# DomhnallBoyle/lip2speech-unit

Measured on AMD Instinct MI355X. Metric: real-time factor (audio-sec/wall-sec), end-to-end lip->16kHz audio, 4s@25fps clips, higher is better.
Workload: dtype fp16; 1 GPU; e2e lip->units->wav (BASELINE configs[3]: AV-HuBERT large 24L + conformer 12x512 + multi_input HiFi-GAN), 4-s 100-frame 88x88 clips, batch 640 per GPU; clips_per_gpu=640, streams=1, clips_per_launch=640, frames_per_clip=100, hipgraph=True, input=uint8 96x96 frames resident in HBM, crop+normalise on device, enc_layers=24, conf_layers=12, parallelism=clip-parallel dp1

## Files before the change

include/lip2speech_hip.h:

```cpp
#ifndef LIP2SPEECH_HIP_H
#define LIP2SPEECH_HIP_H

#include <stddef.h>
#include <stdint.h>

#ifdef __cplusplus
extern "C" {
#endif

#define L2S_ABI_VERSION 16

enum { L2S_F16 = 0, L2S_BF16 = 1, L2S_F32 = 2 };

enum { L2S_OK = 0, L2S_EINVAL = -1, L2S_ESHAPE = -2, L2S_EALIGN = -3, L2S_EUNSUPPORTED = -4 };

enum {
  L2S_ACT_NONE = 0,
  L2S_ACT_RELU = 1,
  L2S_ACT_GELU = 2,
  L2S_ACT_SWISH = 3,
  L2S_ACT_PRELU = 4,
  L2S_ACT_LRELU = 5,
  L2S_ACT_TANH = 6
};

enum {
  L2S_F_RES_PRE  = 1 << 0,
  L2S_F_RES_POST = 1 << 1,
  L2S_F_ACCUM    = 1 << 2,
  L2S_F_DUAL     = 1 << 3,
  L2S_F_MASK     = 1 << 4,
  L2S_F_OUT_F32  = 1 << 5,
  L2S_F_RES_F32  = 1 << 6
};

enum {
  L2S_MODE_LINEAR = 0,
  L2S_MODE_CONV1D = 1,
  L2S_MODE_CONV2D = 2
};

typedef struct l2s_gemm_desc {
  const void* A;
  const void* W;
  void* C;
  void* C2;
  const float* bias;
  const float* slope;
  const void* R;
  const int32_t* lens;
  int32_t M, N, Cin, ntaps;
  int32_t lda, ldc, ldc2, ldr;
  int32_t mode;
  int32_t T_out, T_in, stride, dil, off;
  int32_t Ho, Wo, Hi, Wi, KW, pad;
  int32_t out_row_mul, out_row_add;
  int32_t mask_T, mask_mul;
  int32_t act, flags, dtype;
  float alpha;
  float act_slope;
  float slope2;
  int32_t groups, a_gstride, c_gstride;
  int64_t w_gstride;
  const int32_t* ktab;
} l2s_gemm_desc;
#define L2S_KTAB_MAX 9

int l2s_abi_version(void);
const char* l2s_build_info(void);

int l2s_tapgemm(const l2s_gemm_desc* host_desc, void* stream);
#define L2S_VARIANT_F32 2128128
int l2s_tapgemm_variant(const l2s_gemm_desc* host_desc);
#define L2S_EPI_FAMILY_F32 32
int l2s_tapgemm_epilogue_family(const l2s_gemm_desc* host_desc);

int l2s_stem_conv3d(const void* x, int x_is_f32, const void* w, const float* bias, const float* slope,
                    void* y, int B, int T, int H, int W, int dtype, void* stream);

int l2s_stem_pool_fused(const void* x, int x_is_f32, const void* w, const float* bias, const float* slope,
                        void* y, int B, int T, int H, int W, int dtype, void* stream);

int l2s_stem_pool_fused_u8(const uint8_t* frames, int Hin, int Win, int crop, float mean, float std, const void* w,
                           const float* bias, const float* slope, void* y, int B, int T, int dtype, void* stream);

int l2s_maxpool2d_3x3s2(const void* x, void* y, int N, int H, int W, int C, int dtype, void* stream);

int l2s_avgpool_hw(const void* x, void* y, int N, int HW, int C, int dtype, void* stream);

int l2s_layernorm(const void* x, int x_is_f32, int ldx, const float* gamma, const float* beta, float eps,
                  void* y, int y_is_f32, int ldy, void* y2, int ldy2, int M, int C, int zero_prefix,
                  const int32_t* lens, int len_mul, int mask_T, int dtype, void* stream);

int l2s_attention(const void* qkv, int ldq, void* out, int ldo, const void* pos, int ldp,
                  const float* bias_u, const float* bias_v, const int32_t* lens, int len_mul,
                  int B, int T, int H, int dtype, void* stream);

int l2s_glu_dwconv_swish(const void* x, const float* w, const float* bias, void* y, const int32_t* lens,
                         int len_mul, int B, int T, int C, int k, int dtype, void* stream);

int l2s_greedy_decode(const float* logits, int ldl, const int32_t* lens, int len_mul, int B, int T2, int V,
                      float temperature, float lenpen, int32_t* tokens, float* lprobs, float* score, void* stream);

int l2s_beam_decode(const float* logits, int ldl, const int32_t* lens, int len_mul, int B, int T2, int V, float temperature,
                    float lenpen, int beam, void* workspace, size_t workspace_bytes, int32_t* tokens, float* pos_scores,
                    float* score, int32_t* nhyp, void* stream);
size_t l2s_beam_decode_workspace(int B, int T2, int beam);

int l2s_ctc_frames(const float* logits, int ldl, const int32_t* lens, int len_mul, int B, int L, int V, int K, int32_t* labels,
                   int32_t* topk_cls, float* topk_lp, void* stream);

int l2s_ctc_beam_search(const int32_t* topk_cls, const float* topk_lp, const int32_t* lens, int len_mul, int B, int L, int K,
                        int beam, int nbest, void* workspace, size_t workspace_bytes, int32_t* labels, int32_t* lengths,
                        float* scores, void* stream);
size_t l2s_ctc_beam_workspace(int B, int L, int beam);
int l2s_ctc_repeat_labels(const int32_t* x, int ldx, const int32_t* lens, int len_mul, int B, int L, int32_t* y, int ldy,
                          void* stream);

int l2s_repeat2_cast(const float* x, void* y, int B, int T, int C, int dtype, void* stream);

int l2s_splitk_reduce(const float* P, int ldp, int S, float* x, int ldx, int M, int N, void* stream);

int l2s_splitk_reduce_layernorm(const float* P, int ldp, int S, float* x, int ldx, const float* gamma, const float* beta, float eps,
                                void* y, int y_is_f32, int ldy, int M, int C, const int32_t* lens, int len_mul, int mask_T,
                                int dtype, void* stream);

int l2s_cast_f32_to_16(const float* x, int ldx, void* y, int ldy, int M, int C, int dtype, void* stream);
int l2s_cast_16_to_f32(const void* x, int ldx, float* y, int ldy, int M, int C, int dtype, void* stream);
int l2s_broadcast_rows(const void* v, int ldv, void* y, int ldy, int col0, const int32_t* lens, int len_mul,
                       int B, int T, int C, int v_is_f32, int dtype, void* stream);
int l2s_transpose_ct_to_tc(const float* x, void* y, int ldy, int col0, const int32_t* lens, int len_mul,
                           int B, int C, int T, int dtype, void* stream);
int l2s_embedding(const int32_t* code, const void* table, void* y, int ldy, const int32_t* lens,
                  int B, int L, int C, int dtype, void* stream);
int l2s_embedding_tokens(const int32_t* tok, int ldt, int token_offset, const void* table, int n_rows, void* y, int ldy,
                         const int32_t* lens, int len_mul, int B, int L, int C, int dtype, void* stream);
int l2s_rows_f32_to_16_masked(const float* x, int ldx, void* y, int ldy, int col0, const int32_t* lens, int len_mul,
                              int B, int T, int C, int dtype, void* stream);
int l2s_lens_from_mask(const uint8_t* mask, int32_t* lens, int B, int T, void* stream);
int l2s_split_hi_lo(const float* x, int ldx, void* hi, void* lo, int ld16, int act, float slope, const int32_t* lens,
                    int len_mul, int B, int T, int C, int dtype, void* stream);

typedef struct l2s_respair_desc {
  const void* X; const void* W1; const void* W2; const float* b1; const float* b2;
  void* Y; float* XS; const int32_t* lens;
  int32_t len_mul, B, T, C, k, dil, last, accumulate, dtype;
  float slope;
} l2s_respair_desc;
int l2s_respair(const l2s_respair_desc* d, void* stream);

typedef struct l2s_respair_final_desc {
  const void* X[3]; const void* W1[3]; const void* W2[3]; const float* b1[3]; const float* b2[3];
  int32_t k[3], dil[3];
  void* Y; const int32_t* lens;
  int32_t n, len_mul, B, T, C, dtype;
  float slope;
} l2s_respair_final_desc;
int l2s_respair_final(const l2s_respair_final_desc* d, void* stream);

int l2s_basicblock_fused(const void* x, const void* w1, const float* b1, const float* s1, const void* w2, const float* b2,
                         const float* s2, void* y, int n_images, int H, int W, int C, int dtype, void* stream);
int l2s_basiclayer_fused(const void* x, const void* const* w, const float* const* bias, const float* const* slope, int n_blocks,
                         void* y, int n_images, int H, int W, int C, int dtype, void* stream);
int l2s_basicstage128_tail_fused(const void* x0, const void* t0, const void* wa, const float* ba, const float* sa, const void* w1,
                                 const float* b1, const float* s1, const void* w2, const float* b2, const float* s2, void* y,
                                 int n_images, int H, int W, int dtype, void* stream);

int l2s_conv_post_tanh(const float* x, const float* w, float bias, float* wav, int16_t* pcm, const int32_t* lens,
                       int len_mul, int B, int T, int C, int k, void* stream);

int l2s_resblock_fused(const void* xl, const void* w, const float* bias, float* xs, void* xl_out,
                       const int32_t* lens, int len_mul, int B, int T, int C, int k, int d0, int d1, int d2,
                       int accumulate, float slope, int dtype, void* stream);

int l2s_resstage_fused(const void* xl, const void* const* w, const float* const* bias, const int* ks, const int* dils,
                       int n_blocks, float* xs, void* xl_out, const int32_t* lens, int len_mul, int B, int T, int C,
                       float slope, int xs_final, int dtype, void* stream);

int l2s_preprocess_frames(const uint8_t* frames, void* y, int B, int T, int Hin, int Win, int crop, float mean,
                          float std, int dtype, void* stream);

int l2s_mel_spectrogram(const void* wav, int wav_is_i16, int64_t ldw, const int32_t* n_samples, int B, int S, const float* basis,
                        const float* fb, const int32_t* fb_range, float* mel, int ldm, int T_rows, int n_fft, int hop,
                        int n_mels, float floor_, void* stream);

int l2s_unit_ce(const float* logits, int ldl, const int32_t* target, int ldt, const int32_t* lens, int len_mul, int B, int T2,
                int V, int pad_idx, int ignore_prefix, float* nll, float* smooth, int32_t* n_correct, int32_t* n_tok,
                void* stream);
int l2s_mel_l1_sc(const float* pred, int Tm_pred, const float* targ, int Tm_targ, const int32_t* lens, int len_mul, int B,
                  int n_mels, int crop_len, float* l1, float* sq, float* tsq, int32_t* n_rows, void* stream);
size_t l2s_ctc_loss_workspace(int B, int L, int S_max);
int l2s_ctc_loss(const float* logits, int ldl, const int32_t* lens, int len_mul, int B, int L, int V, int blank,
                 const int32_t* targets, const int32_t* tgt_lens, const int32_t* tgt_offs, int S_max, void* workspace,
                 size_t workspace_bytes, float* nll, void* stream);

#ifdef __cplusplus
}
#endif
#endif
```

lip2speech_unit_amd/_lib.py:

```python
import ctypes
import os

_HERE = os.path.dirname(os.path.abspath(__file__))
LIB_PATH = os.environ.get("L2S_LIB_PATH") or os.path.join(_HERE, "liblip2speech_hip.so")

F16, BF16, F32 = 0, 1, 2
ACT_NONE, ACT_RELU, ACT_GELU, ACT_SWISH, ACT_PRELU, ACT_LRELU, ACT_TANH = range(7)
F_RES_PRE, F_RES_POST, F_ACCUM, F_DUAL, F_MASK, F_OUT_F32, F_RES_F32 = (1 << i for i in range(7))
MODE_LINEAR, MODE_CONV1D, MODE_CONV2D = 0, 1, 2
ABI_VERSION = 16

_ERR = {-1: "L2S_EINVAL", -2: "L2S_ESHAPE", -3: "L2S_EALIGN", -4: "L2S_EUNSUPPORTED"}


class L2SError(RuntimeError):
    pass


class GemmDesc(ctypes.Structure):
    _fields_ = [
        ("A", ctypes.c_void_p), ("W", ctypes.c_void_p), ("C", ctypes.c_void_p), ("C2", ctypes.c_void_p),
        ("bias", ctypes.c_void_p), ("slope", ctypes.c_void_p), ("R", ctypes.c_void_p), ("lens", ctypes.c_void_p),
        ("M", ctypes.c_int32), ("N", ctypes.c_int32), ("Cin", ctypes.c_int32), ("ntaps", ctypes.c_int32),
        ("lda", ctypes.c_int32), ("ldc", ctypes.c_int32), ("ldc2", ctypes.c_int32), ("ldr", ctypes.c_int32),
        ("mode", ctypes.c_int32),
        ("T_out", ctypes.c_int32), ("T_in", ctypes.c_int32), ("stride", ctypes.c_int32), ("dil", ctypes.c_int32),
        ("off", ctypes.c_int32),
        ("Ho", ctypes.c_int32), ("Wo", ctypes.c_int32), ("Hi", ctypes.c_int32), ("Wi", ctypes.c_int32),
        ("KW", ctypes.c_int32), ("pad", ctypes.c_int32),
        ("out_row_mul", ctypes.c_int32), ("out_row_add", ctypes.c_int32),
        ("mask_T", ctypes.c_int32), ("mask_mul", ctypes.c_int32),
        ("act", ctypes.c_int32), ("flags", ctypes.c_int32), ("dtype", ctypes.c_int32),
        ("alpha", ctypes.c_float), ("act_slope", ctypes.c_float), ("slope2", ctypes.c_float),
        ("groups", ctypes.c_int32), ("a_gstride", ctypes.c_int32), ("c_gstride", ctypes.c_int32),
        ("w_gstride", ctypes.c_int64),
        ("ktab", ctypes.c_void_p),
    ]


_vp, _i, _f = ctypes.c_void_p, ctypes.c_int, ctypes.c_float


class RespairDesc(ctypes.Structure):
    _fields_ = [("X", ctypes.c_void_p), ("W1", ctypes.c_void_p), ("W2", ctypes.c_void_p), ("b1", ctypes.c_void_p),
                ("b2", ctypes.c_void_p), ("Y", ctypes.c_void_p), ("XS", ctypes.c_void_p), ("lens", ctypes.c_void_p),
                ("len_mul", ctypes.c_int32), ("B", ctypes.c_int32), ("T", ctypes.c_int32), ("C", ctypes.c_int32),
                ("k", ctypes.c_int32), ("dil", ctypes.c_int32), ("last", ctypes.c_int32), ("accumulate", ctypes.c_int32),
                ("dtype", ctypes.c_int32), ("slope", ctypes.c_float)]


class RespairFinalDesc(ctypes.Structure):
    _fields_ = [("X", ctypes.c_void_p * 3), ("W1", ctypes.c_void_p * 3), ("W2", ctypes.c_void_p * 3), ("b1", ctypes.c_void_p * 3),
                ("b2", ctypes.c_void_p * 3), ("k", ctypes.c_int32 * 3), ("dil", ctypes.c_int32 * 3),
                ("Y", ctypes.c_void_p), ("lens", ctypes.c_void_p),
                ("n", ctypes.c_int32), ("len_mul", ctypes.c_int32), ("B", ctypes.c_int32), ("T", ctypes.c_int32),
                ("C", ctypes.c_int32), ("dtype", ctypes.c_int32), ("slope", ctypes.c_float)]


SIGNATURES = {
    "l2s_abi_version": ([], ctypes.c_int),
    "l2s_build_info": ([], ctypes.c_char_p),
    "l2s_tapgemm": ([ctypes.POINTER(GemmDesc), _vp], _i),
    "l2s_tapgemm_variant": ([ctypes.POINTER(GemmDesc)], _i),
    "l2s_tapgemm_epilogue_family": ([ctypes.POINTER(GemmDesc)], _i),
    "l2s_stem_conv3d": ([_vp, _i, _vp, _vp, _vp, _vp, _i, _i, _i, _i, _i, _vp], _i),
    "l2s_stem_pool_fused": ([_vp, _i, _vp, _vp, _vp, _vp, _i, _i, _i, _i, _i, _vp], _i),
    "l2s_stem_pool_fused_u8": ([_vp, _i, _i, _i, _f, _f, _vp, _vp, _vp, _vp, _i, _i, _i, _vp], _i),
    "l2s_maxpool2d_3x3s2": ([_vp, _vp, _i, _i, _i, _i, _i, _vp], _i),
    "l2s_avgpool_hw": ([_vp, _vp, _i, _i, _i, _i, _vp], _i),
    "l2s_layernorm": ([_vp, _i, _i, _vp, _vp, _f, _vp, _i, _i, _vp, _i, _i, _i, _i, _vp, _i, _i, _i, _vp], _i),
    "l2s_attention": ([_vp, _i, _vp, _i, _vp, _i, _vp, _vp, _vp, _i, _i, _i, _i, _i, _vp], _i),
    "l2s_glu_dwconv_swish": ([_vp, _vp, _vp, _vp, _vp, _i, _i, _i, _i, _i, _i, _vp], _i),
    "l2s_greedy_decode": ([_vp, _i, _vp, _i, _i, _i, _i, _f, _f, _vp, _vp, _vp, _vp], _i),
    "l2s_beam_decode": ([_vp, _i, _vp, _i, _i, _i, _i, _f, _f, _i, _vp, ctypes.c_size_t, _vp, _vp, _vp, _vp, _vp], _i),
    "l2s_beam_decode_workspace": ([_i, _i, _i], ctypes.c_size_t),
    "l2s_ctc_frames": ([_vp, _i, _vp, _i, _i, _i, _i, _i, _vp, _vp, _vp, _vp], _i),
    "l2s_ctc_beam_search": ([_vp, _vp, _vp, _i, _i, _i, _i, _i, _i, _vp, ctypes.c_size_t, _vp, _vp, _vp, _vp], _i),
    "l2s_ctc_beam_workspace": ([_i, _i, _i], ctypes.c_size_t),
    "l2s_ctc_repeat_labels": ([_vp, _i, _vp, _i, _i, _i, _vp, _i, _vp], _i),
    "l2s_repeat2_cast": ([_vp, _vp, _i, _i, _i, _i, _vp], _i),
    "l2s_splitk_reduce": ([_vp, _i, _i, _vp, _i, _i, _i, _vp], _i),
    "l2s_splitk_reduce_layernorm": ([_vp, _i, _i, _vp, _i, _vp, _vp, _f, _vp, _i, _i, _i, _i, _vp, _i, _i, _i, _vp], _i),
    "l2s_cast_f32_to_16": ([_vp, _i, _vp, _i, _i, _i, _i, _vp], _i),
    "l2s_cast_16_to_f32": ([_vp, _i, _vp, _i, _i, _i, _i, _vp], _i),
    "l2s_broadcast_rows": ([_vp, _i, _vp, _i, _i, _vp, _i, _i, _i, _i, _i, _i, _vp], _i),
    "l2s_transpose_ct_to_tc": ([_vp, _vp, _i, _i, _vp, _i, _i, _i, _i, _i, _vp], _i),
    "l2s_embedding": ([_vp, _vp, _vp, _i, _vp, _i, _i, _i, _i, _vp], _i),
    "l2s_embedding_tokens": ([_vp, _i, _i, _vp, _i, _vp, _i, _vp, _i, _i, _i, _i, _i, _vp], _i),
    "l2s_rows_f32_to_16_masked": ([_vp, _i, _vp, _i, _i, _vp, _i, _i, _i, _i, _i, _vp], _i),
    "l2s_lens_from_mask": ([_vp, _vp, _i, _i, _vp], _i),
    "l2s_basicblock_fused": ([_vp, _vp, _vp, _vp, _vp, _vp, _vp, _vp, _i, _i, _i, _i, _i, _vp], _i),
    "l2s_basiclayer_fused": ([_vp, _vp, _vp, _vp, _i, _vp, _i, _i, _i, _i, _i, _vp], _i),
    "l2s_basicstage128_tail_fused": ([_vp] * 12 + [_i, _i, _i, _i, _vp], _i),
    "l2s_split_hi_lo": ([_vp, _i, _vp, _vp, _i, _i, _f, _vp, _i, _i, _i, _i, _i, _vp], _i),
    "l2s_conv_post_tanh": ([_vp, _vp, _f, _vp, _vp, _vp, _i, _i, _i, _i, _i, _vp], _i),
    "l2s_resblock_fused": ([_vp, _vp, _vp, _vp, _vp, _vp, _i, _i, _i, _i, _i, _i, _i, _i, _i, _f, _i, _vp], _i),
    "l2s_resstage_fused": ([_vp, _vp, _vp, _vp, _vp, _i, _vp, _vp, _vp, _i, _i, _i, _i, _f, _i, _i, _vp], _i),
    "l2s_respair": ([ctypes.POINTER(RespairDesc), _vp], _i),
    "l2s_respair_final": ([ctypes.POINTER(RespairFinalDesc), _vp], _i),
    "l2s_preprocess_frames": ([_vp, _vp, _i, _i, _i, _i, _i, _f, _f, _i, _vp], _i),
    "l2s_mel_spectrogram": ([_vp, _i, ctypes.c_int64, _vp, _i, _i, _vp, _vp, _vp, _vp, _i, _i, _i, _i, _i, _f, _vp], _i),
    "l2s_unit_ce": ([_vp, _i, _vp, _i, _vp, _i, _i, _i, _i, _i, _i, _vp, _vp, _vp, _vp, _vp], _i),
    "l2s_mel_l1_sc": ([_vp, _i, _vp, _i, _vp, _i, _i, _i, _i, _vp, _vp, _vp, _vp, _vp], _i),
    "l2s_ctc_loss_workspace": ([_i, _i, _i], ctypes.c_size_t),
    "l2s_ctc_loss": ([_vp, _i, _vp, _i, _i, _i, _i, _i, _vp, _vp, _vp, _i, _vp, ctypes.c_size_t, _vp, _vp], _i),
}

_lib = None


def load():
    global _lib
    if _lib is not None:
        return _lib
    if not os.path.exists(LIB_PATH):
        raise L2SError(
            f"{LIB_PATH} not found: build it with `python -c 'import __graft_entry__ as g; g.build()'` "
            "(make -C lip2speech_unit_amd/csrc). The MI355X path has no CPU fallback.")
    import torch
    lib = ctypes.CDLL(LIB_PATH)
    for name, (argtypes, restype) in SIGNATURES.items():
        try:
            fn = getattr(lib, name)
        except AttributeError as e:
            raise L2SError(f"{LIB_PATH} does not export {name}; rebuild the library") from e
        fn.argtypes = argtypes
        fn.restype = restype
    v = lib.l2s_abi_version()
    if v != ABI_VERSION:
        raise L2SError(f"ABI mismatch: library {v}, binding {ABI_VERSION}")
    _lib = lib
    return lib


def check(rc, what):
    if rc == 0:
        return
    if rc < 0:
        raise L2SError(f"{what}: rejected with {_ERR.get(rc, rc)}")
    raise L2SError(f"{what}: HIP launch failed with hipError_t={rc}")
```

lip2speech_unit_amd/conformer.py:

```python
import math
import os
from dataclasses import dataclass, field

import torch
import torch.nn as nn

from . import ops
from .ops import ACT_GELU, ACT_RELU, F_MASK, F_RES_POST, MODE_CONV1D


@dataclass
class ConformerConfig:
    conformer_embed_dim: int = 512
    conformer_attention_heads: int = 8
    conformer_ffn_embed_dim: int = 2048
    conformer_layers: int = 12
    cnn_module_kernel: int = 31
    encoder_embed_dim: int = 1024
    decoder_embed_dim: int = 204
    spk_dim: int = 256
    mel_dim: int = 160
    text_supervision: bool = field(default_factory=lambda: bool(int(os.environ.get("TEXT_SUPERVISION", 0))))
    text_classes: int = 4000

    @classmethod
    def from_model_cfg(cls, cfg):
        from .plugin import cfg_get
        c = cls()
        for k in ("conformer_embed_dim", "conformer_attention_heads", "conformer_ffn_embed_dim", "conformer_layers"):
            setattr(c, k, int(cfg_get(cfg, k, getattr(c, k))))
        c.text_supervision = bool(cfg_get(cfg, "text_supervision", c.text_supervision))
        return c


class TextClassifier(nn.Module):

    def __init__(self, d, num_classes):
        super().__init__()
        self.classifier = nn.Linear(d, num_classes)

    def _load_from_state_dict(self, state_dict, prefix, *a, **k):
        w = state_dict.get(prefix + "classifier.weight")
        if w is not None and w.dim() == 2 and w.shape[0] != self.classifier.out_features and w.shape[1] == self.classifier.in_features:
            self.classifier = nn.Linear(w.shape[1], w.shape[0])
        super()._load_from_state_dict(state_dict, prefix, *a, **k)


class PositionwiseFeedForward(nn.Module):
    def __init__(self, d, hidden):
        super().__init__()
        self.w_1 = nn.Linear(d, hidden)
        self.w_2 = nn.Linear(hidden, d)


class RelPositionMultiHeadedAttention(nn.Module):
    def __init__(self, heads, d):
        super().__init__()
        self.h, self.d_k = heads, d // heads
        self.linear_q = nn.Linear(d, d)
        self.linear_k = nn.Linear(d, d)
        self.linear_v = nn.Linear(d, d)
        self.linear_out = nn.Linear(d, d)
        self.linear_pos = nn.Linear(d, d, bias=False)
        self.pos_bias_u = nn.Parameter(torch.zeros(heads, d // heads))
        self.pos_bias_v = nn.Parameter(torch.zeros(heads, d // heads))


class ConvolutionModule(nn.Module):
    def __init__(self, ch, k):
        super().__init__()
        self.pointwise_cov1 = nn.Conv1d(ch, 2 * ch, 1)
        self.depthwise_conv = nn.Conv1d(ch, ch, k, padding=(k - 1) // 2, groups=ch)
        self.norm = nn.BatchNorm1d(ch)
        self.pointwise_cov2 = nn.Conv1d(ch, ch, 1)


class EncoderLayer(nn.Module):
    def __init__(self, d, heads, hidden, k):
        super().__init__()
        self.self_attn = RelPositionMultiHeadedAttention(heads, d)
        self.feed_forward = PositionwiseFeedForward(d, hidden)
        self.conv_module = ConvolutionModule(d, k)
        self.norm_ff = nn.LayerNorm(d, eps=1e-12)
        self.norm_mha = nn.LayerNorm(d, eps=1e-12)
        self.feed_forward_macaron = PositionwiseFeedForward(d, hidden)
        self.norm_ff_macaron = nn.LayerNorm(d, eps=1e-12)
        self.norm_conv = nn.LayerNorm(d, eps=1e-12)
        self.norm_final = nn.LayerNorm(d, eps=1e-12)


class RavenEncoderLayer(nn.Module):

    def __init__(self, d, heads, hidden):
        super().__init__()
        self.self_attn = RelPositionMultiHeadedAttention(heads, d)
        self.feed_forward = PositionwiseFeedForward(d, hidden)
        self.norm_ff = nn.BatchNorm1d(d)
        self.norm_mha = nn.LayerNorm(d, eps=1e-12)
        self.gamma_ff = nn.Parameter(0.1 * torch.ones(d))
        self.gamma_mha = nn.Parameter(0.1 * torch.ones(d))


class Encoder(nn.Module):

    def __init__(self, d, heads, hidden, blocks, k, idim=512, raven=False):
        super().__init__()
        self.frontend = None
        self.raven = raven
        self.embed = nn.Sequential(nn.Linear(idim, d))
        self.encoders = nn.ModuleList([RavenEncoderLayer(d, heads, hidden) if raven else EncoderLayer(d, heads, hidden, k)
                                       for _ in range(blocks)])
        self.after_norm = nn.LayerNorm(d, eps=1e-12)
        self.d, self.heads, self.hidden, self.k = d, heads, hidden, k
        self._packed = None
        self._pos_cache = {}
        if d // heads != 64:
            raise NotImplementedError("the attention kernels are built for 64-dim heads (512/8, 768/12, 1024/16)")

    def pack(self, dev, dtype):
        t16 = ops.torch_dtype(dtype)
        d = self.d
        inv = 1.0 / math.sqrt(d // self.heads)

        def w16(t):
            return t.detach().float().to(dev, t16).contiguous()

        P = {"layers": [], "dtype": dtype}
        P["w_emb"], P["b_emb"] = w16(self.embed[0].weight), _f32(self.embed[0].bias, dev)
        pos_w = []
        for L in self.encoders if self.raven else ():
            a, bn = L.self_attn, L.norm_ff
            g_m, g_f = L.gamma_mha.detach().float(), L.gamma_ff.detach().float()
            sc = bn.weight.detach().float() / torch.sqrt(bn.running_var.detach().float() + bn.eps)
            sh = bn.bias.detach().float() - bn.running_mean.detach().float() * sc
            w1 = L.feed_forward.w_1.weight.detach().float()
            e = {
                "ff": (w16(w1 * sc[None, :]), (w1 @ sh + L.feed_forward.w_1.bias.detach().float()).to(dev).contiguous(),
                       w16(L.feed_forward.w_2.weight.detach().float() * g_f[:, None]),
                       (L.feed_forward.w_2.bias.detach().float() * g_f).to(dev).contiguous()),
                "wqkv": w16(torch.cat([a.linear_q.weight.detach().float() * inv, a.linear_k.weight.detach().float(),
                                       a.linear_v.weight.detach().float()], 0)),
                "bqkv": torch.cat([a.linear_q.bias.detach().float() * inv, a.linear_k.bias.detach().float(),
                                   a.linear_v.bias.detach().float()], 0).to(dev).contiguous(),
                "u": (a.pos_bias_u.detach().float() * inv).to(dev).contiguous(),
                "v": (a.pos_bias_v.detach().float() * inv).to(dev).contiguous(),
                "wo": w16(a.linear_out.weight.detach().float() * g_m[:, None]),
                "bo": (a.linear_out.bias.detach().float() * g_m).to(dev).contiguous(),
                "n_mha": _ln(L.norm_mha, dev),
            }
            pos_w.append(a.linear_pos.weight.detach().float())
            P["layers"].append(e)
        for L in () if self.raven else self.encoders:
            a, c = L.self_attn, L.conv_module
            bn = c.norm
            sc = bn.weight.detach().float() / torch.sqrt(bn.running_var.detach().float() + bn.eps)
            sh = bn.bias.detach().float() - bn.running_mean.detach().float() * sc
            dw = c.depthwise_conv.weight.detach().float()[:, 0, :] * sc[:, None]
            db = c.depthwise_conv.bias.detach().float() * sc + sh
            e = {
                "ffm": (w16(L.feed_forward_macaron.w_1.weight), _f32(L.feed_forward_macaron.w_1.bias, dev),
                        w16(L.feed_forward_macaron.w_2.weight), _f32(L.feed_forward_macaron.w_2.bias, dev)),
                "ff": (w16(L.feed_forward.w_1.weight), _f32(L.feed_forward.w_1.bias, dev),
                       w16(L.feed_forward.w_2.weight), _f32(L.feed_forward.w_2.bias, dev)),
                "wqkv": w16(torch.cat([a.linear_q.weight.detach().float() * inv, a.linear_k.weight.detach().float(),
                                       a.linear_v.weight.detach().float()], 0)),
                "bqkv": torch.cat([a.linear_q.bias.detach().float() * inv, a.linear_k.bias.detach().float(),
                                   a.linear_v.bias.detach().float()], 0).to(dev).contiguous(),
                "u": (a.pos_bias_u.detach().float() * inv).to(dev).contiguous(),
                "v": (a.pos_bias_v.detach().float() * inv).to(dev).contiguous(),
                "wo": w16(a.linear_out.weight), "bo": _f32(a.linear_out.bias, dev),
                "pw1": w16(c.pointwise_cov1.weight[:, :, 0]), "pb1": _f32(c.pointwise_cov1.bias, dev),
                "dw": dw.t().contiguous().to(dev), "db": db.to(dev).contiguous(),
                "pw2": w16(c.pointwise_cov2.weight[:, :, 0]), "pb2": _f32(c.pointwise_cov2.bias, dev),
                "n_ffm": _ln(L.norm_ff_macaron, dev), "n_mha": _ln(L.norm_mha, dev), "n_conv": _ln(L.norm_conv, dev),
                "n_ff": _ln(L.norm_ff, dev), "n_fin": _ln(L.norm_final, dev),
            }
            pos_w.append(a.linear_pos.weight.detach().float())
            P["layers"].append(e)
        P["w_pos"] = w16(torch.cat(pos_w, 0))
        P["n_after"] = _ln(self.after_norm, dev)
        self._packed = P
        self._pos_cache = {}
        return P

    def _pos_proj(self, T, dev):
        key = (T, str(dev))
        if key not in self._pos_cache:
            P, d = self._packed, self.d
            dt = P["dtype"]
            t16 = ops.torch_dtype(dt)
            pe = rel_pos_table(T, d, dev).to(t16).contiguous()
            nl = len(P["layers"])
            out = torch.empty(2 * T - 1, nl * d, device=dev, dtype=t16)
            ops.tapgemm(pe, P["w_pos"], out, M=2 * T - 1, N=nl * d, Cin=d, dtype=dt)
            self._pos_cache[key] = out
        return self._pos_cache[key]

    def forward_rows(self, xin, lens, B, T, len_mul, dtype):
        dev = xin.device
        if self._packed is None or self._packed["b_emb"].device != dev or self._packed["dtype"] != dtype:
            self.pack(dev, dtype)
        P, dt = self._packed, dtype
        t16 = ops.torch_dtype(dt)
        d, H, F, k = self.d, self.heads, self.hidden, self.k
        M = B * T
        nl = len(P["layers"])
        x = torch.empty(M, d, device=dev, dtype=torch.float32)
        ops.tapgemm(xin, P["w_emb"], x, M=M, N=d, Cin=xin.shape[1], bias=P["b_emb"], alpha=math.sqrt(d), dtype=dt)
        pos = self._pos_proj(T, dev)
        h = torch.empty(M, d, device=dev, dtype=t16)
        f = torch.empty(M, F, device=dev, dtype=t16)
        qkv = torch.empty(M, 3 * d, device=dev, dtype=t16)
        att = torch.empty(M, d, device=dev, dtype=t16)
        glu_in = torch.empty(M, 2 * d, device=dev, dtype=t16)
        cv = torch.empty(M, d, device=dev, dtype=t16)

        def half_ffn(e, name, norm, after, y):
            w = e[name]
            ops.layernorm(x, norm[0], norm[1], 1e-12, h, M=M, C=d, dtype=dt)
            ops.tapgemm(h, w[0], f, M=M, N=F, Cin=d, bias=w[1], act=ACT_RELU, dtype=dt)
            ops.residual_linear(f, w[2], w[3], x, M=M, N=d, K=F, alpha=0.5, dtype=dt, cache=e, key=name,
                                ln=(after[0], after[1], 1e-12, y))

        for li, e in enumerate(P["layers"] if self.raven else ()):
            ops.layernorm(x, e["n_mha"][0], e["n_mha"][1], 1e-12, h, M=M, C=d, dtype=dt)
            ops.tapgemm(h, e["wqkv"], qkv, M=M, N=3 * d, Cin=d, bias=e["bqkv"], dtype=dt)
            ops.attention(qkv, att, B=B, T=T, H=H, pos=pos[:, li * d:], ldp=nl * d, bias_u=e["u"], bias_v=e["v"],
                          lens=lens, len_mul=len_mul, dtype=dt)
            ops.tapgemm(att, e["wo"], x, M=M, N=d, Cin=d, bias=e["bo"], R=x, ldr=d, flags=F_RES_POST, dtype=dt)
            ops.cast_f32_to_16(x, h, M, d, dt)
            w = e["ff"]
            ops.tapgemm(h, w[0], f, M=M, N=F, Cin=d, bias=w[1], act=ACT_RELU, dtype=dt)
            ops.tapgemm(f, w[2], x, M=M, N=d, Cin=F, bias=w[3], R=x, ldr=d, flags=F_RES_POST, dtype=dt)
        for li, e in enumerate(() if self.raven else P["layers"]):
            half_ffn(e, "ffm", e["n_ffm"], e["n_mha"], h)
            ops.tapgemm(h, e["wqkv"], qkv, M=M, N=3 * d, Cin=d, bias=e["bqkv"], dtype=dt)
            ops.attention(qkv, att, B=B, T=T, H=H, pos=pos[:, li * d:], ldp=nl * d, bias_u=e["u"], bias_v=e["v"],
                          lens=lens, len_mul=len_mul, dtype=dt)
            ops.tapgemm(att, e["wo"], x, M=M, N=d, Cin=d, bias=e["bo"], R=x, ldr=d, flags=F_RES_POST, dtype=dt)
            ops.layernorm(x, e["n_conv"][0], e["n_conv"][1], 1e-12, h, M=M, C=d, dtype=dt)
            ops.tapgemm(h, e["pw1"], glu_in, M=M, N=2 * d, Cin=d, bias=e["pb1"], dtype=dt)
            ops.glu_dwconv_swish(glu_in, e["dw"], e["db"], cv, B=B, T=T, C=d, k=k, lens=lens, len_mul=len_mul, dtype=dt)
            ops.tapgemm(cv, e["pw2"], x, M=M, N=d, Cin=d, bias=e["pb2"], R=x, ldr=d, flags=F_RES_POST, dtype=dt)
            half_ffn(e, "ff", e["n_ff"], e["n_fin"], x)
        return x


def _f32(t, dev):
    return t.detach().float().to(dev).contiguous()


def _ln(m, dev):
    return (_f32(m.weight, dev), _f32(m.bias, dev))


def rel_pos_table(T, d, dev):
    rel = torch.arange(T - 1, -T, -1, dtype=torch.float32).unsqueeze(1)
    div = torch.exp(torch.arange(0, d, 2, dtype=torch.float32) * -(math.log(10000.0) / d))
    pe = torch.zeros(2 * T - 1, d)
    pe[:, 0::2] = torch.sin(rel * div)
    pe[:, 1::2] = torch.cos(rel * div)
    return pe.to(dev)


class Conformer(nn.Module):

    def __init__(self, cfg: ConformerConfig = None, dtype=ops.F16):
        super().__init__()
        cfg = cfg or ConformerConfig()
        self.cfg = cfg
        d = cfg.conformer_embed_dim
        self.encoder = Encoder(d, cfg.conformer_attention_heads, cfg.conformer_ffn_embed_dim, cfg.conformer_layers,
                               cfg.cnn_module_kernel)
        self.proj_in = nn.Linear(cfg.encoder_embed_dim, d) if cfg.encoder_embed_dim != d else None
        self.proj_out = nn.Linear(d, cfg.decoder_embed_dim) if cfg.decoder_embed_dim != d else None
        self.mel_conv = nn.Sequential(
            nn.Conv1d(d + cfg.spk_dim, d, 3, 1, 1), nn.Dropout(0.0), nn.GELU(),
            nn.Conv1d(d, d, 3, 1, 1), nn.Dropout(0.0), nn.GELU(),
            nn.Conv1d(d, d, 3, 1, 1), nn.Dropout(0.0), nn.GELU())
        self.mel_proj = nn.Linear(d, cfg.mel_dim)
        self.text_classifier = TextClassifier(d, cfg.text_classes) if cfg.text_supervision else None
        self.dtype = dtype
        self._packed = None

    @property
    def _pos_cache(self):
        return self.encoder._pos_cache

    @_pos_cache.setter
    def _pos_cache(self, v):
        self.encoder._pos_cache = v

    def load_state_dict(self, *a, **k):
        r = super().load_state_dict(*a, **k)
        self._packed = None
        self.encoder._packed, self.encoder._pos_cache = None, {}
        return r

    def pack(self, dev):
        t16 = ops.torch_dtype(self.dtype)
        cfg = self.cfg

        def w16(t):
            return t.detach().float().to(dev, t16).contiguous()

        P = {}
        if self.proj_in is not None:
            P["w_in"], P["b_in"] = w16(self.proj_in.weight), _f32(self.proj_in.bias, dev)
        self.encoder.pack(dev, self.dtype)
        P["n_after"] = self.encoder._packed["n_after"]
        P["mel"] = []
        for i in (0, 3, 6):
            cv = self.mel_conv[i]
            P["mel"].append((w16(cv.weight.detach().permute(0, 2, 1).reshape(cv.weight.shape[0], -1)),
                             _f32(cv.bias, dev), cv.weight.shape[1]))
        D = cfg.mel_dim
        perm = torch.tensor([2 * k + j for j in range(2) for k in range(D // 2)])
        P["w_mel"], P["b_mel"] = w16(self.mel_proj.weight.detach()[perm]), _f32(self.mel_proj.bias.detach()[perm], dev)
        if self.proj_out is not None:
            P["w_out"], P["b_out"] = w16(self.proj_out.weight), _f32(self.proj_out.bias, dev)
        if self.text_classifier is not None:
            lin = self.text_classifier.classifier
            V = lin.out_features
            Vp = -(-V // 4) * 4
            w = torch.zeros(Vp, lin.in_features)
            w[:V] = lin.weight.detach().float().cpu()
            b = torch.full((Vp,), -torch.finfo(torch.float32).max)
            b[:V] = lin.bias.detach().float().cpu()
            P["w_text"], P["b_text"], P["v_text"] = w16(w), b.to(dev).contiguous(), V
        P["dev_probe"] = P["b_mel"]
        self._packed = P

    def forward_rows(self, src16, lens, B, T, spk_emb, len_mul=2):
        dev = src16.device
        if self._packed is None or self._packed["dev_probe"].device != dev:
            self.pack(dev)
        P, dt, cfg = self._packed, self.dtype, self.cfg
        t16 = ops.torch_dtype(dt)
        d = cfg.conformer_embed_dim
        M = B * T
        if self.proj_in is not None:
            xin = torch.empty(M, d, device=dev, dtype=t16)
            ops.tapgemm(src16, P["w_in"], xin, M=M, N=d, Cin=src16.shape[1], bias=P["b_in"], dtype=dt)
        else:
            xin = src16
        x = self.encoder.forward_rows(xin, lens, B, T, len_mul, dt)
        y16 = torch.empty(M, d, device=dev, dtype=t16)
        cat = torch.empty(M, d + cfg.spk_dim, device=dev, dtype=t16)
        ops.layernorm(x, P["n_after"][0], P["n_after"][1], 1e-12, y16, M=M, C=d, dtype=dt)
        ops.layernorm(x, P["n_after"][0], P["n_after"][1], 1e-12, cat[:, cfg.spk_dim:], M=M, C=d, ldy=d + cfg.spk_dim,
                      lens=lens, len_mul=len_mul, mask_T=T, dtype=dt)
        assert spk_emb.size(-1) == cfg.spk_dim
        spk = spk_emb.contiguous()
        if spk.dtype not in (torch.float32, t16):
            spk = spk.float()
        ops.broadcast_rows(spk, cat, B=B, T=T, C=cfg.spk_dim, ldy=d + cfg.spk_dim, col0=0, lens=lens, len_mul=len_mul,
                           dtype=dt)
        cur = cat
        for (w, b, cin) in P["mel"]:
            nxt = torch.empty(M, d, device=dev, dtype=t16)
            ops.tapgemm(cur, w, nxt, M=M, N=d, Cin=cin, ntaps=3, mode=MODE_CONV1D, T_out=T, T_in=T, stride=1, dil=1,
                        off=-1, bias=b, act=ACT_GELU, lens=lens, mask_T=T, mask_mul=len_mul, flags=F_MASK, dtype=dt)
            cur = nxt
        mel = torch.empty(M, cfg.mel_dim, device=dev, dtype=torch.float32)
        ops.tapgemm(cur, P["w_mel"], mel, M=M, N=cfg.mel_dim, Cin=d, bias=P["b_mel"], dtype=dt)
        if self.proj_out is not None:
            V = cfg.decoder_embed_dim
            logits = torch.empty(M, V, device=dev, dtype=torch.float32)
            ops.tapgemm(y16, P["w_out"], logits, M=M, N=V, Cin=d, bias=P["b_out"], dtype=dt)
        else:
            logits = None
        return logits, mel, y16

    @property
    def text_classes(self):
        return self.text_classifier.classifier.out_features if self.text_classifier is not None else 0

    def text_rows(self, y16):
        if self.text_classifier is None:
            raise RuntimeError("this conformer has no text head (TEXT_SUPERVISION=0)")
        dev = y16.device
        if self._packed is None or self._packed["dev_probe"].device != dev:
            self.pack(dev)
        P, d = self._packed, self.cfg.conformer_embed_dim
        M, Vp = y16.shape[0], P["w_text"].shape[0]
        out = torch.empty(M, Vp, device=dev, dtype=torch.float32)
        ops.tapgemm(y16, P["w_text"], out, M=M, N=Vp, Cin=d, bias=P["b_text"], dtype=self.dtype)
        return out

    def forward(self, source, padding_mask, spk_emb=None, tbc=True, **kwargs):
        x = source.transpose(0, 1) if tbc else source
        B, T, C = x.shape
        dev = x.device
        t16 = ops.torch_dtype(self.dtype)
        src16 = x.to(t16).contiguous().view(B * T, C)
        lens = ops.lens_from_mask(None if padding_mask is None else padding_mask.to(torch.bool).contiguous(), B, T, dev)
        if spk_emb is None:
            raise NotImplementedError("the mel head of the released checkpoints is built with the 256-d speaker embedding")
        logits, mel, y16 = self.forward_rows(src16, lens, B, T, spk_emb, len_mul=1)
        V = logits.shape[1]
        unit = logits.view(B, T, V)
        unit = unit.transpose(0, 1) if tbc else unit
        out = {"encoder_out": unit, "encoder_padding_mask": padding_mask, "padding_mask": padding_mask,
               "encoder_out_mel": mel.view(B, 2 * T, self.cfg.mel_dim // 2)}
        if self.text_classifier is not None:
            text = self.text_rows(y16)[:, : self.text_classes].reshape(B, T, -1)
            out["encoder_out_text"] = text.transpose(0, 1) if tbc else text
        return out

    def reorder_encoder_out(self, encoder_out, new_order):
        if encoder_out["encoder_out"] is not None:
            encoder_out["encoder_out"] = encoder_out["encoder_out"].index_select(1, new_order)
        for k in ("encoder_padding_mask", "padding_mask"):
            if encoder_out[k] is not None:
                encoder_out[k] = encoder_out[k].index_select(0, new_order)
        return encoder_out

    def max_positions(self):
        return None
```

lip2speech_unit_amd/csrc/phasegemm.hip:

```cpp
#include "l2s_common.h"
#include "tapgemm_tiles.h"
#include <cstdlib>

int l2s_phasegemm_f16_m0(const l2s_gemm_desc& d, hipStream_t st);
int l2s_phasegemm_f16_m1(const l2s_gemm_desc& d, hipStream_t st);
int l2s_phasegemm_f16_m2(const l2s_gemm_desc& d, hipStream_t st);
int l2s_phasegemm_bf16_m0(const l2s_gemm_desc& d, hipStream_t st);
int l2s_phasegemm_bf16_m1(const l2s_gemm_desc& d, hipStream_t st);
int l2s_phasegemm_bf16_m2(const l2s_gemm_desc& d, hipStream_t st);
int l2s_phasegemm_f16_m3(const l2s_gemm_desc& d, hipStream_t st);
int l2s_phasegemm_bf16_m3(const l2s_gemm_desc& d, hipStream_t st);

int l2s_phasegemm_ktab_launch(const l2s_gemm_desc& d, hipStream_t st) {
  if (d.mode != L2S_MODE_LINEAR || d.groups < 1) return L2S_EINVAL;
  const int fam = l2s::pick_epilogue(d.flags, d.act);
  if (fam != 2 && fam != l2s::L2S_EPI_G16A) return L2S_EUNSUPPORTED;
  if ((d.Cin % 64) || d.N < 256 || d.M < 256 || (d.M & 7) || (d.N & 7) || (d.lda & 7) || (d.ldc & 7) || (d.c_gstride & 63) ||
      (d.ldr & 7) || d.out_row_mul != 1 || d.out_row_add != 0)
    return L2S_EUNSUPPORTED;
  return d.dtype == L2S_F16 ? l2s_phasegemm_f16_m3(d, st) : l2s_phasegemm_bf16_m3(d, st);
}

bool l2s_phasegemm_eligible(const l2s_gemm_desc& d) {
  static const int mode = [] { const char* e = getenv("L2S_PHASEGEMM"); return e ? atoi(e) : 1; }();
  if (mode == 0) return false;
  if (d.groups > 1 || d.mode < 0 || d.mode > 2 || d.ktab) return false;
  if (d.mode == L2S_MODE_LINEAR && d.ntaps != 1) return false;
  if (d.mode == L2S_MODE_CONV1D && (d.T_out <= 0 || d.T_in <= 0)) return false;
  if (d.mode == L2S_MODE_CONV2D && (d.Ho <= 0 || d.Wo <= 0 || d.KW <= 0 || d.ntaps % d.KW)) return false;
  const int fam = l2s::pick_epilogue(d.flags, d.act);
  if (fam == l2s::L2S_EPI_ALL && !(l2s::is_x32(d.flags, d.act) && !(d.ldc & 3) && !(d.ldr & 3) && !(d.ldc2 & 3))) return false;
  static const int res_on = [] { const char* e = getenv("L2S_PHASEGEMM_RES"); return e ? atoi(e) : 1; }();
  if (!res_on && (fam == l2s::L2S_EPI_G16A || fam == l2s::L2S_EPI_G16B)) return false;
  if (fam == l2s::L2S_EPI_S32 && ((d.ldc & 3) || (d.ldr & 3))) return false;
  if ((d.Cin % 64) || d.N < 256 || d.M < 256 || (d.lda & 7)) return false;
  if (d.mode == L2S_MODE_LINEAR && ((d.M & 7) || (d.N & 7))) return false;
  if (mode == 2) return true;
  auto cdivl = [](long a, long b) { return (a + b - 1) / b; };
  const long tm = cdivl(d.M, 256);
  const long rounds_big = cdivl(tm * cdivl(d.N, 256), 256);
  if (rounds_big * ((long)d.Cin * d.ntaps / 64) < 20) return false;
  const double big = (double)rounds_big * 2.0 / 1.2;
  const double reg = (double)cdivl(tm * cdivl(d.N, 128), 256);
  return big < reg;
}

#ifdef L2S_WITH_WIDEGEMM
int l2s_widegemm_f16(const l2s_gemm_desc& d, hipStream_t st);
int l2s_widegemm_bf16(const l2s_gemm_desc& d, hipStream_t st);
static bool wide_ok(const l2s_gemm_desc& d) {
  static const int mode = [] { const char* e = getenv("L2S_WIDEGEMM"); return e ? atoi(e) : 0; }();
  if (mode == 0 || d.mode != L2S_MODE_LINEAR) return false;
  const int fam = l2s::pick_epilogue(d.flags, d.act);
  if (fam > l2s::L2S_EPI_G16A && fam != l2s::L2S_EPI_S32) return false;
  return !(d.M & 7) && !(d.N & 7);
}
#endif

int l2s_phasegemm_launch(const l2s_gemm_desc& d, hipStream_t st) {
  const bool h = d.dtype == L2S_F16;
#ifdef L2S_WITH_WIDEGEMM
  if (wide_ok(d)) return h ? l2s_widegemm_f16(d, st) : l2s_widegemm_bf16(d, st);
#endif
  switch (d.mode) {
    case L2S_MODE_LINEAR: return h ? l2s_phasegemm_f16_m0(d, st) : l2s_phasegemm_bf16_m0(d, st);
    case L2S_MODE_CONV1D: return h ? l2s_phasegemm_f16_m1(d, st) : l2s_phasegemm_bf16_m1(d, st);
    case L2S_MODE_CONV2D: return h ? l2s_phasegemm_f16_m2(d, st) : l2s_phasegemm_bf16_m2(d, st);
    default: return L2S_EINVAL;
  }
}
```

lip2speech_unit_amd/csrc/phasegemm_inst.hip:

```cpp
#include "phasegemm_kernel.h"

#define L2S_PCAT_(a, b) a##b
#define L2S_PCAT(a, b) L2S_PCAT_(a, b)
#if L2S_INST_ET == 0
using InstET = ElemF16;
#define L2S_INST_NAME L2S_PCAT(l2s_phasegemm_f16_m, L2S_INST_MODE)
#else
using InstET = ElemBF16;
#define L2S_INST_NAME L2S_PCAT(l2s_phasegemm_bf16_m, L2S_INST_MODE)
#endif

int L2S_INST_NAME(const l2s_gemm_desc& d, hipStream_t st) { return launch_phase_mode<InstET, L2S_INST_MODE>(d, st); }

#if defined(L2S_PHASE_STAMPS) && L2S_INST_ET == 0 && L2S_INST_MODE == 0
extern "C" int l2s_debug_phase_stamps(void* buf) { return phase_set_stamps(buf); }
#endif
```

lip2speech_unit_amd/csrc/phasegemm_kernel.h:

```cpp
#pragma once
#include "tapgemm_common.h"
#include <cstdlib>

using namespace l2s;

namespace {

constexpr int PBM = 256, PBN = 256, PBK = 64;
constexpr int Q_B = 128 * PBK * 2;
constexpr bool p_generic(int epi) { return epi == L2S_EPI_G16A || epi == L2S_EPI_G16B; }
constexpr int p_scr_b(int epi) { return p_generic(epi) ? 16 * 64 * 4 : 16 * (4 * 32 + 16); }
constexpr int p_smem(int epi) { return 8 * Q_B + 8 * p_scr_b(epi); }

#ifdef L2S_PHASE_STAMPS
__device__ unsigned long long* g_phase_stamps = nullptr;
#define PHSTAMP(i) { const unsigned long long now_ = __builtin_amdgcn_s_memtime(); ph_acc[i] += now_ - ph_last; ph_last = now_; }
#else
#define PHSTAMP(i)
#endif

constexpr int PG_KTAB = 3;
template <typename ET, int MODE_T, int EPI>
__global__ __launch_bounds__(512) void phasegemm_kernel(const l2s_gemm_desc p, const int tilesM, const int tilesN,
                                                        const int chunk, const int band) {
  constexpr bool KT = MODE_T == PG_KTAB;
  constexpr int MODE = KT ? (int)L2S_MODE_LINEAR : MODE_T;
  constexpr int MI = 8, NI = 4;
#ifdef L2S_NO_PAIRED
  constexpr bool PAIRED = false;
#else
  constexpr bool PAIRED = EPI <= L2S_EPI_G16A;
#endif
  extern __shared__ __attribute__((aligned(16))) uint16_t lds[];
  const int tid = threadIdx.x, lane = tid & 63;
  const int wave = __builtin_amdgcn_readfirstlane(tid >> 6);
  const int wr = wave >> 2, wc = wave & 3;
  const int K = p.Cin * p.ntaps;
  const int nk = K / PBK;
  const uint16_t* zero = reinterpret_cast<const uint16_t*>(&g_zero16);

  const int tiles_mn = tilesM * tilesN;
  const int ntiles = tiles_mn * (KT ? p.groups : 1);
  const int slot = blockIdx.x >> 3, slots = gridDim.x >> 3;
  const int lo = (blockIdx.x & 7) * chunk;
  const int hi = lo + chunk < ntiles ? lo + chunk : ntiles;
  const int my_n = (lo + slot < hi) ? (hi - lo - slot + slots - 1) / slots : 0;
  if (my_n == 0) return;
  const int total_q = my_n * nk * 4;
  auto tile_coords = [&](int i, int& m0, int& n0, int& g) {
    int l = lo + slot + i * slots;
    g = 0;
    if constexpr (KT) {
      const int per_m = p.groups * tilesN;
      const int mt = l / per_m, r = l - mt * per_m;
      g = r / tilesN;
      m0 = mt * PBM;
      n0 = (r - g * tilesN) * PBN;
      return;
    }
    const int bsz = band * tilesN;
    const int bi = l / bsz, idx = l - bi * bsz;
    const int rows = tilesM - bi * band < band ? tilesM - bi * band : band;
    const int tn = idx / rows;
    m0 = (bi * band + idx - tn * rows) * PBM;
    n0 = tn * PBN;
  };

  const int srow = lane >> 3;
  const int schunk = (lane & 7) ^ (srow & 7);
  const uint16_t* qa_ptr[2][2];
  int qa_t[2][2], qa_x[2][2];
  const uint16_t* qb_ptr[2][2];
  int run_tap = 0, run_c = 0, run_ky = 0, run_kx = 0;
  const char* sa_base[2][2] = {{nullptr, nullptr}, {nullptr, nullptr}};
  const char* sw_base[2][2] = {{nullptr, nullptr}, {nullptr, nullptr}};
  uint32_t a_lane = 0, w_lane[2] = {0, 0};
  if constexpr (MODE == L2S_MODE_LINEAR) {
    a_lane = (uint32_t)(srow * p.lda * 2 + (schunk << 4));
#pragma unroll
    for (int j = 0; j < 2; ++j) {
      const int within = 16 * (wave & 1) + 8 * j + srow;
      const int bchunk = PAIRED ? ((lane & 7) ^ paired_w_key(within)) : schunk;
      w_lane[j] = (uint32_t)(srow * K * 2 + (bchunk << 4));
    }
  }
  typedef const int32_t __attribute__((address_space(4)))* ktab_ptr_t;
  constexpr int KTN = L2S_KTAB_MAX;
  const ktab_ptr_t kt_tab = (ktab_ptr_t)(uintptr_t)p.ktab;
  ktab_ptr_t kt_row = kt_tab;
  int nk_stage = nk, kt_blk = 0, kt_win = 0;
  uint32_t kt_cur_a = 0, kt_cur_w = 0, kt_nxt_a = 0, kt_nxt_w = 0;
  const int kpb = KT ? p.Cin / PBK : 1;
  auto setup_issue = [&](int i) {
    int m0, n0, tg;
    tile_coords(i, m0, n0, tg);
    if constexpr (KT) {
      kt_row = kt_tab + tg * (2 + 2 * KTN);
      nk_stage = kt_row[0] * kpb;
      kt_blk = 0; kt_win = 0;
      kt_cur_a = (uint32_t)kt_row[2] * 2u; kt_cur_w = (uint32_t)kt_row[2 + KTN] * 2u;
      kt_nxt_a = (uint32_t)kt_row[3] * 2u; kt_nxt_w = (uint32_t)kt_row[3 + KTN] * 2u;
    }
#ifdef L2S_ABL_SAMETILE
    m0 = 0; n0 = 0;
#endif
    if constexpr (MODE == L2S_MODE_LINEAR) {
#pragma unroll
      for (int h = 0; h < 2; ++h)
#pragma unroll
        for (int j = 0; j < 2; ++j) {
          int mg = m0 + (wave >> 2) * 128 + h * 64 + 16 * (wave & 3) + 8 * j;
          mg = mg < p.M ? mg : p.M - 8;
          sa_base[h][j] = (const char*)p.A + (int64_t)mg * p.lda * 2;
          int ng = n0 + (wave >> 1) * 64 + h * 32 + 16 * (wave & 1) + 8 * j;
          ng = ng < p.N ? ng : p.N - 8;
          sw_base[h][j] = (const char*)p.W + (int64_t)ng * K * 2;
        }
      return;
    }
#pragma unroll
    for (int h = 0; h < 2; ++h)
#pragma unroll
      for (int j = 0; j < 2; ++j) {
        int m = m0 + (wave >> 2) * 128 + h * 64 + 16 * (wave & 3) + 8 * j + srow;
        m = m < p.M ? m : p.M - 1;
        qa_t[h][j] = 0; qa_x[h][j] = 0;
        if (MODE == L2S_MODE_LINEAR) {
          qa_ptr[h][j] = (const uint16_t*)p.A + (int64_t)m * p.lda + schunk * 8;
        } else if (MODE == L2S_MODE_CONV1D) {
          const int b = m / p.T_out, t = m - b * p.T_out;
          qa_ptr[h][j] = (const uint16_t*)p.A + (int64_t)b * p.T_in * p.lda + schunk * 8;
          qa_t[h][j] = t * p.stride + p.off;
        } else {
          const int hw = p.Ho * p.Wo;
          const int img = m / hw, rem = m - img * hw;
          const int oy = rem / p.Wo, ox = rem - oy * p.Wo;
          qa_ptr[h][j] = (const uint16_t*)p.A + (int64_t)img * p.Hi * p.Wi * p.lda + schunk * 8;
          qa_t[h][j] = oy * p.stride - p.pad;
          qa_x[h][j] = ox * p.stride - p.pad;
        }
        const int within = 16 * (wave & 1) + 8 * j + srow;
        int n = n0 + (wave >> 1) * 64 + h * 32 + within;
        n = n < p.N ? n : p.N - 1;
        const int bchunk = PAIRED ? ((lane & 7) ^ paired_w_key(within)) : schunk;
        qb_ptr[h][j] = (const uint16_t*)p.W + (int64_t)n * K + bchunk * 8;
      }
  };
  auto slot_off = [&](int b, int e) -> uint32_t { return (uint32_t)((b * 4 + e) * Q_B); };
  int s_i = 0, s_kt = 0, s_e = 0, s_par = 0, staged = 0;
  auto stage_one = [&](auto e_tag) {
    constexpr int E = decltype(e_tag)::value;
    const bool live = staged < total_q;
    const int k0 = s_kt * PBK;
    const int se = E >= 0 ? E : s_e;
    uint16_t* dst = lds + (slot_off(s_par, se) >> 1) + wave * 1024;
    const bool is_a = (se == 0) || (se == 3);
    const int h = (se == 2 || se == 3) ? 1 : 0;
    if constexpr (MODE == L2S_MODE_LINEAR) {
      static_assert(E >= 0, "LINEAR stages with a compile-time element");
      const uint32_t kb = (uint32_t)k0 * 2u;
      const uint32_t kba = KT ? kt_cur_a : kb, kbw = KT ? kt_cur_w : kb;
#pragma unroll
      for (int j = 0; j < 2; ++j) {
        const char* g = is_a ? sa_base[h][j] + (size_t)kba + (size_t)a_lane : sw_base[h][j] + (size_t)kbw + (size_t)w_lane[j];
#ifdef L2S_ABL_ZEROSRC
        g = (const char*)zero;
#endif
#if defined(L2S_ABL_WARMDMA)
        if (staged < 8) __builtin_amdgcn_global_load_lds((gptr_t)g, (lptr_t)(dst + j * 512), 16, 0, 0);
#elif !defined(L2S_ABL_NODMA)
        __builtin_amdgcn_global_load_lds((gptr_t)g, (lptr_t)(dst + j * 512), 16, 0, 0);
#endif
      }
      return;
    }
#pragma unroll
    for (int j = 0; j < 2; ++j) {
      const uint16_t* g;
      bool ok = live;
      if (!is_a) {
        g = qb_ptr[h][j] + k0;
      } else if (MODE == L2S_MODE_LINEAR) {
        g = qa_ptr[h][j] + k0;
      } else if (MODE == L2S_MODE_CONV1D) {
        const int st = qa_t[h][j] + run_tap * p.dil;
        ok = ok && ((unsigned)st < (unsigned)p.T_in);
        g = qa_ptr[h][j] + (st * p.lda + run_c);
      } else {
        const int iy = qa_t[h][j] + run_ky, ix = qa_x[h][j] + run_kx;
        ok = ok && ((unsigned)iy < (unsigned)p.Hi) && ((unsigned)ix < (unsigned)p.Wi);
        g = qa_ptr[h][j] + ((iy * p.Wi + ix) * p.lda + run_c);
      }
      g = ok ? g : zero;
#ifdef L2S_ABL_ZEROSRC
      g = zero;
#endif
#ifndef L2S_ABL_NODMA
      __builtin_amdgcn_global_load_lds((gptr_t)g, (lptr_t)(dst + j * 512), 16, 0, 0);
#endif
    }
  };
  auto stage_advance = [&]() {
    const bool live = staged < total_q;
    ++staged;
    if constexpr (MODE == L2S_MODE_LINEAR) {
      if (++s_e == 4) {
        s_e = 0;
        s_par ^= 1;
        if constexpr (KT) {
          if (!(s_i + 1 == my_n && s_kt + 1 == nk_stage)) {
            if (++s_kt == nk_stage) {
              s_kt = 0;
              setup_issue(++s_i);
            } else if (++kt_win == kpb) {
              kt_win = 0;
              ++kt_blk;
              kt_cur_a = kt_nxt_a; kt_cur_w = kt_nxt_w;
              const int nb = kt_blk + 1 < KTN ? kt_blk + 1 : KTN - 1;
              kt_nxt_a = (uint32_t)kt_row[2 + nb] * 2u; kt_nxt_w = (uint32_t)kt_row[2 + KTN + nb] * 2u;
            } else {
              kt_cur_a += PBK * 2; kt_cur_w += PBK * 2;
            }
          }
        } else if (staged < total_q && ++s_kt == nk) {
          s_kt = 0;
          setup_issue(++s_i);
        }
      }
      return;
    }
    if (++s_e == 4) {
      s_e = 0;
      s_par ^= 1;
      if (MODE != L2S_MODE_LINEAR) {
        run_c += PBK;
        if (run_c >= p.Cin) {
          run_c = 0;
          ++run_tap;
          if (++run_kx == p.KW) { run_kx = 0; ++run_ky; }
        }
      }
      if (live && ++s_kt == nk) {
        s_kt = 0;
        run_tap = 0; run_c = 0; run_ky = 0; run_kx = 0;
        if (++s_i < my_n) setup_issue(s_i);
      }
    }
  };

  const int lm = lane & 15, lg = lane >> 4;
  const uint32_t lds_base = (uint32_t)(uintptr_t)(lptr_t)lds;
  const uint32_t k0_off = (uint32_t)(lm * 128 + (((0 + lg) ^ (lm & 7)) << 4));
  const uint32_t k1_off = (uint32_t)(lm * 128 + (((4 + lg) ^ (lm & 7)) << 4));
  const uint32_t a_row = (uint32_t)(wr * 64) * 128;
  const uint32_t b_row = (uint32_t)(wc * 32) * 128;
  frag16 fa[4][2], fb[2][2][2];
  auto read_a = [&](uint32_t qbase) {
    const uint32_t a0 = qbase + a_row + k0_off, a1 = qbase + a_row + k1_off;
    lds_read_b128<0>(fa[0][0], a0); lds_read_b128<2048>(fa[1][0], a0); lds_read_b128<4096>(fa[2][0], a0); lds_read_b128<6144>(fa[3][0], a0);
    lds_read_b128<0>(fa[0][1], a1); lds_read_b128<2048>(fa[1][1], a1); lds_read_b128<4096>(fa[2][1], a1); lds_read_b128<6144>(fa[3][1], a1);
  };
  uint32_t bk_off[2][2];
#pragma unroll
  for (int s2 = 0; s2 < 2; ++s2)
#pragma unroll
    for (int ks = 0; ks < 2; ++ks)
      bk_off[s2][ks] = PAIRED ? paired_w_off(lm, s2, 4 * ks + lg) : (uint32_t)(s2 * 2048) + (ks ? k1_off : k0_off);
  auto read_b = [&](frag16(&f)[2][2], uint32_t qbase) {
    const uint32_t b = qbase + b_row;
    lds_read_b128<0>(f[0][0], b + bk_off[0][0]); lds_read_b128<0>(f[1][0], b + bk_off[1][0]);
    lds_read_b128<0>(f[0][1], b + bk_off[0][1]); lds_read_b128<0>(f[1][1], b + bk_off[1][1]);
  };

  f32x4_t acc[MI][NI];
#pragma unroll
  for (int i = 0; i < MI; ++i)
#pragma unroll
    for (int j = 0; j < NI; ++j) acc[i][j] = f32x4_t{0.f, 0.f, 0.f, 0.f};

  setup_issue(0);
  stage_one(std::integral_constant<int, 0>{}); stage_advance();
  stage_one(std::integral_constant<int, 1>{}); stage_advance();
  stage_one(std::integral_constant<int, 2>{}); stage_advance();
  stage_one(std::integral_constant<int, 3>{}); stage_advance();
  stage_one(std::integral_constant<int, 0>{}); stage_advance();
  stage_one(std::integral_constant<int, 1>{}); stage_advance();
  wait_vmcnt<8>();
  __builtin_amdgcn_s_barrier();
  if (wr == 1) __builtin_amdgcn_s_barrier();

  auto phase = [&](auto q_tag, const int par) {
    constexpr int Q = decltype(q_tag)::value;
#ifndef L2S_ABL_NOREAD
    if (Q == 0) { read_b(fb[0], lds_base + slot_off(par, 1)); __builtin_amdgcn_sched_barrier(0); read_a(lds_base + slot_off(par, 0)); }
    if (Q == 1) read_b(fb[1], lds_base + slot_off(par, 2));
    if (Q == 2) read_a(lds_base + slot_off(par, 3));
#endif
    stage_one(std::integral_constant<int, (Q + 2) & 3>{});
    __builtin_amdgcn_sched_barrier(0);
    wait_vmcnt<8>();
    asm volatile("" ::: "memory");
    __builtin_amdgcn_s_barrier();
    asm volatile("" ::: "memory");
    lds_wait();
    __builtin_amdgcn_s_setprio(1);
    constexpr int RH = (Q >= 2) ? 1 : 0, CH = (Q == 1 || Q == 2) ? 1 : 0;
#ifdef L2S_ABL_MFMA32
    {
      typedef __attribute__((ext_vector_type(16))) float f32x16_t;
#pragma unroll
      for (int mb = 0; mb < 2; ++mb) {
        f32x16_t c;
#pragma unroll
        for (int e = 0; e < 16; ++e) c[e] = acc[RH * 4 + mb * 2 + (e >> 3)][CH * 2 + ((e >> 2) & 1)][e & 3];
#pragma unroll
        for (int kk = 0; kk < 4; ++kk)
          c = __builtin_amdgcn_mfma_f32_32x32x16_f16(fb[CH][kk >> 1][kk & 1].h, fa[mb * 2 + (kk >> 1)][kk & 1].h, c, 0, 0, 0);
#pragma unroll
        for (int e = 0; e < 16; ++e) acc[RH * 4 + mb * 2 + (e >> 3)][CH * 2 + ((e >> 2) & 1)][e & 3] = c[e];
      }
    }
#elif !defined(L2S_ABL_NOMFMA)
#pragma unroll
    for (int i = 0; i < 4; ++i)
#pragma unroll
      for (int j = 0; j < 2; ++j) {
        acc[RH * 4 + i][CH * 2 + j] = ET::mfma(fb[CH][j][0], fa[i][0], acc[RH * 4 + i][CH * 2 + j]);
        acc[RH * 4 + i][CH * 2 + j] = ET::mfma(fb[CH][j][1], fa[i][1], acc[RH * 4 + i][CH * 2 + j]);
      }
#endif
    __builtin_amdgcn_s_setprio(0);
    __builtin_amdgcn_sched_barrier(0);
    asm volatile("" ::: "memory");
    __builtin_amdgcn_s_barrier();
    asm volatile("" ::: "memory");
    __builtin_amdgcn_sched_barrier(0);
    stage_advance();
  };

  int par = 0;
#ifdef L2S_PHASE_STAMPS
  unsigned long long ph_acc[4] = {0, 0, 0, 0};
  unsigned long long ph_last = __builtin_amdgcn_s_memtime();
  const unsigned long long ph_t0 = ph_last;
#endif
  auto nk_of = [&](int ti) -> int {
    if (ti >= my_n) return 0;
    const int l = lo + slot + ti * slots;
    const int per_m = p.groups * tilesN;
    return kt_tab[((l % per_m) / tilesN) * (2 + 2 * KTN)] * kpb;
  };
  int nk_next = KT ? nk_of(0) : nk;
  for (int ti = 0; ti < my_n; ++ti) {
    const int nk_c = nk_next;
    if constexpr (KT) nk_next = nk_of(ti + 1);
    for (int kt = 0; kt < nk_c; ++kt) {
#ifdef L2S_PHASE_STAMPS
      if (kt == 1) PHSTAMP(2)
#endif
      phase(std::integral_constant<int, 0>{}, par);
      phase(std::integral_constant<int, 1>{}, par);
      phase(std::integral_constant<int, 2>{}, par);
      phase(std::integral_constant<int, 3>{}, par);
      par ^= 1;
    }
    PHSTAMP(0)
    int m0, n0, grp;
    tile_coords(ti, m0, n0, grp);
    const uint32_t scr = lds_base + 8 * Q_B + (uint32_t)wave * p_scr_b(EPI);
    auto rowmap = [&](int m) -> int64_t { return m < p.M ? (int64_t)m * p.out_row_mul + p.out_row_add : (int64_t)-1; };
    if constexpr (EPI == L2S_EPI_X32) {
      epilogue_stream32x<ET, MI, NI>(p, acc, lane, m0 + wr * 128, n0 + wc * 64, rowmap);
    } else if constexpr (EPI == L2S_EPI_S32) {
      epilogue_direct32<ET, MI, NI>(p, acc, lane, m0 + wr * 128, n0 + wc * 64, grp, rowmap);
    } else if constexpr (PAIRED) {
      epilogue_direct16<ET, MI, NI, EPI, decltype(rowmap), NoHook, true>(p, acc, lane, m0 + wr * 128, n0 + wc * 64, grp, rowmap);
    } else if constexpr (EPI == L2S_EPI_G16A) {
      epilogue_impl<ET, MI, NI, F_G16A, true, true>(p, acc, scr, lane, m0 + wr * 128, n0 + wc * 64, grp, rowmap);
    } else if constexpr (EPI == L2S_EPI_G16B) {
      epilogue_impl<ET, MI, NI, F_G16B, true, true>(p, acc, scr, lane, m0 + wr * 128, n0 + wc * 64, grp, rowmap);
    } else {
      epilogue_fast16<ET, MI, NI, (EPI - L2S_EPI_F16) / 2, ((EPI - L2S_EPI_F16) & 1) != 0, 1>(
          p, acc, scr, lane, m0 + wr * 128, n0 + wc * 64, grp, rowmap);
    }
#pragma unroll
    for (int i = 0; i < MI; ++i)
#pragma unroll
      for (int j = 0; j < NI; ++j) acc[i][j] = f32x4_t{0.f, 0.f, 0.f, 0.f};
    PHSTAMP(1)
  }
  wait_vmcnt<0>();
#ifdef L2S_PHASE_STAMPS
  if (lane == 0 && (wave == 0 || wave == 7) && g_phase_stamps) {
    unsigned long long* o = g_phase_stamps + ((int64_t)blockIdx.x * 2 + (wave ? 1 : 0)) * 8;
    for (int i = 0; i < 3; ++i) o[i] = ph_acc[i];
    o[3] = (unsigned long long)my_n;
    o[4] = __builtin_amdgcn_s_memtime() - ph_t0;
    o[5] = (unsigned long long)nk;
  }
#endif
}

template <typename ET, int MODE, int EPI>
int launch_phase(const l2s_gemm_desc& d, hipStream_t st) {
  auto kern = phasegemm_kernel<ET, MODE, EPI>;
  static L2sSmemOptIn opt_in;
  if (int e = l2s_smem_opt_in(kern, p_smem(EPI), opt_in)) return e;
  const int tilesM = (d.M + PBM - 1) / PBM, tilesN = (d.N + PBN - 1) / PBN;
  const int ntiles = tilesM * tilesN * (MODE == PG_KTAB ? d.groups : 1);
  const int chunk = (ntiles + 7) / 8;
  const int slots = chunk < 32 ? chunk : 32;
  const double ap = (double)PBM * d.Cin * 2.0, wp = (double)PBN * d.Cin * d.ntaps * 2.0;
  auto cdivi = [](int a, int b) { return (a + b - 1) / b; };
  int band = 1;
  double best = 1e300;
  for (int b = 1; b <= tilesM; ++b) {
    const int wn = cdivi(chunk, b) < tilesN ? cdivi(chunk, b) : tilesN;
    const int an = b * cdivi(chunk, b * tilesN);
    const double fp = ap * (an < tilesM ? an : tilesM) + wp * wn;
    if (fp < best) { best = fp; band = b; }
  }
  hipLaunchKernelGGL(kern, dim3(8 * slots), dim3(512), p_smem(EPI), st, d, tilesM, tilesN, chunk, band);
  L2S_CHECK_LAUNCH();
  return L2S_OK;
}


#ifdef L2S_PHASE_STAMPS
int phase_set_stamps(void* buf) { return (int)hipMemcpyToSymbol(HIP_SYMBOL(g_phase_stamps), &buf, sizeof(buf)); }
#endif

template <typename ET, int MODE>
int launch_phase_mode(const l2s_gemm_desc& d, hipStream_t st) {
  if constexpr (MODE == PG_KTAB) {
    switch (pick_epilogue(d.flags, d.act)) {
      case 2: return launch_phase<ET, MODE, 2>(d, st);
      case L2S_EPI_G16A: return launch_phase<ET, MODE, L2S_EPI_G16A>(d, st);
      default: return L2S_EUNSUPPORTED;
    }
  } else {
    switch (pick_epilogue(d.flags, d.act)) {
      case 0: return launch_phase<ET, MODE, 0>(d, st);
      case 1: return launch_phase<ET, MODE, 1>(d, st);
      case 2: return launch_phase<ET, MODE, 2>(d, st);
      case 3: return launch_phase<ET, MODE, 3>(d, st);
      case 4: return launch_phase<ET, MODE, 4>(d, st);
      case 5: return launch_phase<ET, MODE, 5>(d, st);
      case L2S_EPI_G16A: return launch_phase<ET, MODE, L2S_EPI_G16A>(d, st);
      case L2S_EPI_G16B: return launch_phase<ET, MODE, L2S_EPI_G16B>(d, st);
      case L2S_EPI_S32: return launch_phase<ET, MODE, L2S_EPI_S32>(d, st);
      case L2S_EPI_ALL: return is_x32(d.flags, d.act) ? launch_phase<ET, MODE, L2S_EPI_X32>(d, st) : (int)L2S_EUNSUPPORTED;
      default: return L2S_EUNSUPPORTED;
    }
  }
}

}
```

lip2speech_unit_amd/hubert.py:

```python
from dataclasses import dataclass

import torch
import torch.nn as nn

from . import ops
from .ops import ACT_GELU, F_DUAL, F_MASK, F_RES_POST, MODE_CONV1D
from .resnet import ResEncoder


@dataclass
class AVHubertConfig:
    encoder_layers: int = 24
    encoder_embed_dim: int = 1024
    encoder_ffn_embed_dim: int = 4096
    encoder_attention_heads: int = 16
    conv_pos: int = 128
    conv_pos_groups: int = 16
    layer_norm_first: bool = True
    audio_feat_dim: int = 104
    modality_fuse: str = "concat"
    resnet_relu_type: str = "prelu"
    sub_encoder_layers: int = 0

    @classmethod
    def from_w2v_args(cls, w2v_args):
        from .plugin import cfg_get
        m = cfg_get(w2v_args, "model", None)
        if m is None:
            if any(cfg_get(w2v_args, k, None) is not None for k in ("encoder_layers", "encoder_embed_dim")):
                m = w2v_args
            else:
                raise ValueError("w2v_args carries neither a `model` group nor flat encoder fields (encoder_layers, encoder_embed_dim)")
        c = cls()
        for k, v in list(vars(c).items()):
            got = cfg_get(m, k, v)
            if isinstance(v, bool):
                if isinstance(got, str):
                    if got.strip().lower() not in ("true", "false", "1", "0"):
                        raise ValueError(f"w2v_args.model.{k}: cannot read {got!r} as a bool")
                    got = got.strip().lower() in ("true", "1")
                setattr(c, k, bool(got))
            else:
                setattr(c, k, type(v)(got))
        return c


class MultiheadAttention(nn.Module):

    def __init__(self, dim, heads):
        super().__init__()
        self.embed_dim, self.num_heads = dim, heads
        self.k_proj = nn.Linear(dim, dim)
        self.v_proj = nn.Linear(dim, dim)
        self.q_proj = nn.Linear(dim, dim)
        self.out_proj = nn.Linear(dim, dim)


class TransformerSentenceEncoderLayer(nn.Module):
    def __init__(self, dim, ffn, heads):
        super().__init__()
        self.self_attn = MultiheadAttention(dim, heads)
        self.self_attn_layer_norm = nn.LayerNorm(dim, eps=1e-5)
        self.fc1 = nn.Linear(dim, ffn)
        self.fc2 = nn.Linear(ffn, dim)
        self.final_layer_norm = nn.LayerNorm(dim, eps=1e-5)


class _WeightNormConv1d(nn.Module):

    def __init__(self, cin, cout, k, groups):
        super().__init__()
        self.weight_g = nn.Parameter(torch.ones(1, 1, k))
        self.weight_v = nn.Parameter(torch.zeros(cout, cin // groups, k))
        self.bias = nn.Parameter(torch.zeros(cout))


class TransformerEncoder(nn.Module):

    def __init__(self, cfg: AVHubertConfig, dtype=ops.F16):
        super().__init__()
        d = cfg.encoder_embed_dim
        self.cfg = cfg
        self.pos_conv = nn.Sequential(_WeightNormConv1d(d, d, cfg.conv_pos, cfg.conv_pos_groups))
        self.layers = nn.ModuleList(
            [TransformerSentenceEncoderLayer(d, cfg.encoder_ffn_embed_dim, cfg.encoder_attention_heads)
             for _ in range(cfg.encoder_layers)])
        self.layer_norm = nn.LayerNorm(d, eps=1e-5)
        self.dtype = dtype
        self._packed = None
        if not cfg.layer_norm_first:
            raise NotImplementedError("only layer_norm_first=True (AV-HuBERT large) is built")

    def pack(self, dev):
        t16 = ops.torch_dtype(self.dtype)
        cfg = self.cfg
        d, G, k = cfg.encoder_embed_dim, cfg.conv_pos_groups, cfg.conv_pos
        pc = self.pos_conv[0]
        g, v = pc.weight_g.detach().float(), pc.weight_v.detach().float()
        w = v * (g / v.pow(2).sum(dim=(0, 1), keepdim=True).sqrt())
        cg = d // G
        P = {"pc_w": w.view(G, cg, cg, k).permute(0, 1, 3, 2).reshape(G, cg, k * cg).to(dev, t16).contiguous(),
             "pc_b": pc.bias.detach().float().to(dev).contiguous(), "layers": []}
        scale = (d // cfg.encoder_attention_heads) ** -0.5
        for L in self.layers:
            a = L.self_attn
            wq = a.q_proj.weight.detach().float() * scale
            bq = a.q_proj.bias.detach().float() * scale
            e = {
                "wqkv": torch.cat([wq, a.k_proj.weight.detach().float(), a.v_proj.weight.detach().float()], 0)
                .to(dev, t16).contiguous(),
                "bqkv": torch.cat([bq, a.k_proj.bias.detach().float(), a.v_proj.bias.detach().float()], 0)
                .to(dev).contiguous(),
                "wo": a.out_proj.weight.detach().to(dev, t16).contiguous(),
                "bo": a.out_proj.bias.detach().float().to(dev).contiguous(),
                "w1": L.fc1.weight.detach().to(dev, t16).contiguous(),
                "b1": L.fc1.bias.detach().float().to(dev).contiguous(),
                "w2": L.fc2.weight.detach().to(dev, t16).contiguous(),
                "b2": L.fc2.bias.detach().float().to(dev).contiguous(),
                "ln1": (L.self_attn_layer_norm.weight.detach().float().to(dev).contiguous(),
                        L.self_attn_layer_norm.bias.detach().float().to(dev).contiguous()),
                "ln2": (L.final_layer_norm.weight.detach().float().to(dev).contiguous(),
                        L.final_layer_norm.bias.detach().float().to(dev).contiguous()),
            }
            P["layers"].append(e)
        P["lnf"] = (self.layer_norm.weight.detach().float().to(dev).contiguous(),
                    self.layer_norm.bias.detach().float().to(dev).contiguous())
        self._packed = P

    def forward_rows(self, x32, x16, lens, B, T):
        dev = x32.device
        if self._packed is None or self._packed["pc_b"].device != dev:
            self.pack(dev)
        P, dt, cfg = self._packed, self.dtype, self.cfg
        t16 = ops.torch_dtype(dt)
        d, H, F = cfg.encoder_embed_dim, cfg.encoder_attention_heads, cfg.encoder_ffn_embed_dim
        G, k = cfg.conv_pos_groups, cfg.conv_pos
        cg = d // G
        M = B * T
        x = torch.empty(M, d, device=dev, dtype=torch.float32)
        ops.tapgemm(x16, P["pc_w"], x, M=M, N=cg, Cin=cg, ntaps=k, lda=d, ldc=d, mode=MODE_CONV1D, T_out=T, T_in=T,
                    stride=1, dil=1, off=-(k // 2), bias=P["pc_b"], act=ACT_GELU, R=x32, ldr=d, flags=F_RES_POST,
                    dtype=dt, groups=G, a_gstride=cg, c_gstride=cg, w_gstride=cg * k * cg)
        h = torch.empty(M, d, device=dev, dtype=t16)
        qkv = torch.empty(M, 3 * d, device=dev, dtype=t16)
        att = torch.empty(M, d, device=dev, dtype=t16)
        f = torch.empty(M, F, device=dev, dtype=t16)
        out = torch.empty(M, d, device=dev, dtype=torch.float32)
        layers = P["layers"]
        if not layers:
            ops.layernorm(x, P["lnf"][0], P["lnf"][1], 1e-5, out, M=M, C=d, dtype=dt)
            return out
        ops.layernorm(x, layers[0]["ln1"][0], layers[0]["ln1"][1], 1e-5, h, M=M, C=d, dtype=dt)
        for li, e in enumerate(layers):
            ops.tapgemm(h, e["wqkv"], qkv, M=M, N=3 * d, Cin=d, bias=e["bqkv"], dtype=dt)
            ops.attention(qkv, att, B=B, T=T, H=H, lens=lens, len_mul=1, dtype=dt)
            ops.residual_linear(att, e["wo"], e["bo"], x, M=M, N=d, K=d, dtype=dt, cache=e, key="wo",
                                ln=(e["ln2"][0], e["ln2"][1], 1e-5, h))
            ops.tapgemm(h, e["w1"], f, M=M, N=F, Cin=d, bias=e["b1"], act=ACT_GELU, dtype=dt)
            last = li + 1 == len(layers)
            nxt = P["lnf"] if last else layers[li + 1]["ln1"]
            ops.residual_linear(f, e["w2"], e["b2"], x, M=M, N=d, K=F, dtype=dt, cache=e, key="w2",
                                ln=(nxt[0], nxt[1], 1e-5, out if last else h))
        return out


class SubModel(nn.Module):

    def __init__(self, resnet=None, input_dim=None, cfg: AVHubertConfig = None):
        super().__init__()
        self.resnet = resnet
        self.proj = nn.Linear(input_dim, cfg.encoder_embed_dim)
        if cfg.sub_encoder_layers > 0:
            raise NotImplementedError("sub_encoder_layers > 0 is not used by AV-HuBERT large")
        self.encoder = None


class AVHubertModel(nn.Module):

    def __init__(self, cfg: AVHubertConfig = None, dtype=ops.F16):
        super().__init__()
        cfg = cfg or AVHubertConfig()
        self.cfg = cfg
        d = cfg.encoder_embed_dim
        resnet = ResEncoder(relu_type=cfg.resnet_relu_type, weights=None, dtype=dtype)
        self.feature_extractor_audio = SubModel(resnet=None, input_dim=cfg.audio_feat_dim, cfg=cfg)
        self.feature_extractor_video = SubModel(resnet=resnet, input_dim=resnet.backend_out, cfg=cfg)
        if cfg.modality_fuse != "concat":
            raise NotImplementedError("modality_fuse='add' is not used by the lip2speech checkpoints")
        self.embed = 2 * d
        self.encoder_embed_dim = d
        self.post_extract_proj = nn.Linear(self.embed, d)
        self.mask_emb = nn.Parameter(torch.zeros(cfg.audio_feat_dim))
        self.encoder = TransformerEncoder(cfg, dtype=dtype)
        self.layer_norm = nn.LayerNorm(self.embed, eps=1e-5)
        self.dtype = dtype
        self._packed = None

    def pack(self, dev):
        t16 = ops.torch_dtype(self.dtype)
        fv = self.feature_extractor_video
        self._packed = {
            "wp": fv.proj.weight.detach().to(dev, t16).contiguous(),
            "bp": fv.proj.bias.detach().float().to(dev).contiguous(),
            "ln": (self.layer_norm.weight.detach().float().to(dev).contiguous(),
                   self.layer_norm.bias.detach().float().to(dev).contiguous()),
            "wpe": self.post_extract_proj.weight.detach().to(dev, t16).contiguous(),
            "bpe": self.post_extract_proj.bias.detach().float().to(dev).contiguous(),
        }
        fv.resnet.pack(dev)
        self.encoder.pack(dev)

    def repack(self):
        self._packed = None
        self.encoder._packed = None
        self.feature_extractor_video.resnet._packed = None

    def load_state_dict(self, *a, **k):
        r = super().load_state_dict(*a, **k)
        self.repack()
        return r

    @staticmethod
    def lens_from_padding_mask(padding_mask, B, T, dev):
        if padding_mask is not None:
            padding_mask = padding_mask.to(torch.bool).contiguous()
        return ops.lens_from_mask(padding_mask, B, T, dev)

    def forward_padding_mask(self, features, padding_mask):
        return padding_mask

    def extract_rows(self, video, padding_mask):
        dev = video.device
        if self._packed is None or self._packed["bp"].device != dev:
            self.pack(dev)
        P, dt = self._packed, self.dtype
        t16 = ops.torch_dtype(dt)
        d = self.encoder_embed_dim
        feat, B, T = self.feature_extractor_video.resnet.forward_rows(video)
        M = B * T
        lens = self.lens_from_padding_mask(padding_mask, B, T, dev)
        fv = torch.empty(M, d, device=dev, dtype=torch.float32)
        ops.tapgemm(feat, P["wp"], fv, M=M, N=d, Cin=feat.shape[1], bias=P["bp"], dtype=dt)
        fused = torch.empty(M, 2 * d, device=dev, dtype=t16)
        ops.layernorm(fv, P["ln"][0], P["ln"][1], 1e-5, fused, M=M, C=d, zero_prefix=d, dtype=dt)
        x32 = torch.empty(M, d, device=dev, dtype=torch.float32)
        x16 = torch.empty(M, d, device=dev, dtype=t16)
        ops.tapgemm(fused, P["wpe"], x32, M=M, N=d, Cin=2 * d, bias=P["bpe"], C2=x16, ldc2=d, lens=lens, mask_T=T,
                    mask_mul=1, flags=F_MASK | F_DUAL, slope2=1.0, dtype=dt)
        out = self.encoder.forward_rows(x32, x16, lens, B, T)
        return out, lens, B, T

    def extract_finetune(self, source, padding_mask=None, mask=False, ret_conv=False, output_layer=None):
        if source.get("audio") is not None:
            raise NotImplementedError("audio modality is outside the lip2speech inference path (modalities=['video'])")
        if mask or ret_conv or output_layer is not None:
            raise NotImplementedError("mask / ret_conv / output_layer are training-time options")
        out, lens, B, T = self.extract_rows(source["video"], padding_mask)
        return out.view(B, T, -1), padding_mask

    def remove_pretraining_modules(self):
        pass


class HubertEncoderWrapper(nn.Module):

    def __init__(self, w2v_model):
        super().__init__()
        self.w2v_model = w2v_model

    def forward(self, source, padding_mask, **kwargs):
        x, padding_mask = self.w2v_model.extract_finetune(source=source, padding_mask=padding_mask)
        return {"encoder_out": x.transpose(0, 1), "encoder_padding_mask": padding_mask, "padding_mask": padding_mask}

    def forward_torchscript(self, net_input):
        return self.forward(**{k: v for k, v in net_input.items() if k in ("source", "padding_mask")})

    def reorder_encoder_out(self, encoder_out, new_order):
        if encoder_out["encoder_out"] is not None:
            encoder_out["encoder_out"] = encoder_out["encoder_out"].index_select(1, new_order)
        for k in ("encoder_padding_mask", "padding_mask"):
            if encoder_out[k] is not None:
                encoder_out[k] = encoder_out[k].index_select(0, new_order)
        return encoder_out

    def max_positions(self):
        return None
```

lip2speech_unit_amd/ops.py:

```python
import ctypes
import os
from typing import Optional

import torch

from . import _lib
from ._lib import (ACT_GELU, ACT_LRELU, ACT_NONE, ACT_PRELU, ACT_RELU, ACT_SWISH, ACT_TANH, BF16, F16, F32, F_ACCUM,
                   F_DUAL, F_MASK, F_OUT_F32, F_RES_F32, F_RES_POST, F_RES_PRE, MODE_CONV1D, MODE_CONV2D,
                   MODE_LINEAR, GemmDesc, L2SError, check)

_TORCH16 = {F16: torch.float16, BF16: torch.bfloat16, F32: torch.float32}
_DTYPE_NAME = {F16: "f16", BF16: "bf16", F32: "f32"}


class KernelProfiler:

    def __init__(self, detail=False):
        self.records = []
        self.detail = detail

    def summary(self):
        torch.cuda.synchronize()
        agg = {}
        for key, fl, by, e0, e1, shape in self.records:
            a = agg.setdefault(key, {"calls": 0, "ms": 0.0, "flops": 0.0, "bytes": 0.0, "shapes": {}})
            ms = e0.elapsed_time(e1)
            for t in (a, a["shapes"].setdefault(shape, {"calls": 0, "ms": 0.0, "flops": 0.0, "bytes": 0.0})):
                t["calls"] += 1
                t["ms"] += ms
                t["flops"] += fl
                t["bytes"] += by
        return agg


_profiler = None


def set_profiler(p):
    global _profiler
    _profiler = p


def _run(key, call, flops=0.0, nbytes=0.0, shape=None):
    if _profiler is None:
        return check(call(), key)
    e0, e1 = torch.cuda.Event(enable_timing=True), torch.cuda.Event(enable_timing=True)
    e0.record()
    rc = call()
    e1.record()
    check(rc, key)
    _profiler.records.append((key, flops, nbytes, e0, e1, shape))


def torch_dtype(dtype: int) -> torch.dtype:
    return _TORCH16[dtype]


def dtype_code(t: torch.dtype) -> int:
    if t == torch.float16:
        return F16
    if t == torch.bfloat16:
        return BF16
    if t == torch.float32:
        return F32
    raise L2SError(f"unsupported operand dtype {t}")


def _stream() -> int:
    return torch.cuda.current_stream().cuda_stream


def _ptr(t: Optional[torch.Tensor]) -> Optional[int]:
    if t is None:
        return None
    if not t.is_cuda:
        raise L2SError("HIP ops need device tensors (there is no CPU path)")
    return t.data_ptr()


def _req(t: torch.Tensor, dtype=None, name="tensor"):
    if not t.is_cuda:
        raise L2SError(f"{name}: expected a device tensor (there is no CPU path)")
    if dtype is not None and t.dtype != dtype:
        raise L2SError(f"{name}: expected {dtype}, got {t.dtype}")
    if t.dim() >= 2 and t.stride(-1) != 1:
        raise L2SError(f"{name}: innermost dim must be contiguous")
    return t


def _extent(t: torch.Tensor) -> int:
    if t.numel() == 0:
        return 0
    return 1 + sum((n - 1) * st for n, st in zip(t.shape, t.stride()))


def tapgemm(A, W, C, *, M, N, Cin, ntaps=1, lda=None, ldc=None, bias=None, slope=None, R=None, ldr=None, C2=None,
            ldc2=None, lens=None, mode=MODE_LINEAR, T_out=0, T_in=0, stride=1, dil=1, off=0, Ho=0, Wo=0, Hi=0, Wi=0,
            KW=1, pad=0, out_row_mul=1, out_row_add=0, mask_T=0, mask_mul=1, act=ACT_NONE, flags=0, dtype=F16,
            alpha=1.0, act_slope=0.0, slope2=0.0, groups=1, a_gstride=0, c_gstride=0, w_gstride=0, ktab=None, kflops=None):
    lib = _lib.load()
    d = GemmDesc()
    d.A, d.W, d.C = _ptr(A), _ptr(W), _ptr(C)
    d.C2, d.bias, d.slope, d.R, d.lens = _ptr(C2), _ptr(bias), _ptr(slope), _ptr(R), _ptr(lens)
    if bias is not None and bias.dtype != torch.float32:
        raise L2SError("bias must be fp32")
    if lens is not None and lens.dtype != torch.int32:
        raise L2SError("lens must be int32")
    d.M, d.N, d.Cin, d.ntaps = M, N, Cin, ntaps
    d.lda = lda if lda is not None else Cin
    d.ldc = ldc if ldc is not None else N * groups
    d.ldc2 = ldc2 if ldc2 is not None else d.ldc
    d.ldr = ldr if ldr is not None else d.ldc
    d.mode = mode
    d.T_out, d.T_in, d.stride, d.dil, d.off = T_out, T_in, stride, dil, off
    d.Ho, d.Wo, d.Hi, d.Wi, d.KW, d.pad = Ho, Wo, Hi, Wi, KW, pad
    d.out_row_mul, d.out_row_add = out_row_mul, out_row_add
    d.mask_T, d.mask_mul = mask_T, mask_mul
    if C.dtype == torch.float32:
        flags |= F_OUT_F32
    if R is not None and R.dtype == torch.float32:
        flags |= F_RES_F32
    d.act, d.flags, d.dtype = act, flags, dtype
    d.alpha, d.act_slope, d.slope2 = alpha, act_slope, slope2
    d.groups, d.a_gstride, d.c_gstride, d.w_gstride = groups, a_gstride, c_gstride, w_gstride
    if ktab is not None:
        if ktab.dtype != torch.int32 or ktab.dim() != 2 or ktab.shape != (groups, 20) or not ktab.is_contiguous():
            raise L2SError("ktab: int32 [groups, 20], contiguous")
        d.ktab = _ptr(ktab)
    if _profiler is None:
        check(lib.l2s_tapgemm(ctypes.byref(d), _stream()), "l2s_tapgemm")
        return
    var = lib.l2s_tapgemm_variant(ctypes.byref(d))
    key = f"tapgemm<{_DTYPE_NAME[dtype]},{var // 1000 % 1000}x{var % 1000},mode{mode}>"
    if _profiler is not None:
        fam = lib.l2s_tapgemm_epilogue_family(ctypes.byref(d))
        if var in (999064, 999128):
            fam = {0: 2, 1: 3, 2: 2, 3: 3, 6: 6, 7: 7}.get(fam, 9)
        key = key[:-1] + f",e{fam}>"
    if _profiler is not None and _profiler.detail:
        key += f" M{M} N{N} Cin{Cin} taps{ntaps} g{groups} fl{flags:#x} act{act} alpha{alpha:g}"
    ktot = Cin * ntaps
    osz = 4 if dtype == F32 else 2
    esz = 4 if (flags & F_OUT_F32) else osz
    mn = float(M) * N * groups
    nbytes = float(osz) * M * ktot * groups / max(ntaps, 1) + float(osz) * N * ktot * groups + esz * mn
    if R is not None:
        nbytes += (4 if (flags & F_RES_F32) else osz) * mn
    if flags & F_DUAL:
        nbytes += osz * mn
    if flags & F_ACCUM:
        nbytes += esz * mn
    _run(key, lambda: lib.l2s_tapgemm(ctypes.byref(d), _stream()), kflops if kflops is not None else 2.0 * M * N * ktot * groups, nbytes,
         shape=f"M{M} N{N * groups} K{ktot}" + (" ktab" if ktab is not None else ""))


def stem_conv3d(x, w, bias, slope, y, B, T, dtype):
    lib = _lib.load()
    _run("l2s_stem_conv3d", lambda: lib.l2s_stem_conv3d(_ptr(x), int(x.dtype == torch.float32), _ptr(w), _ptr(bias), _ptr(slope), _ptr(y), B, T,
                              x.shape[-2], x.shape[-1], dtype, _stream()))


def stem_pool_fused(x, w, bias, slope, y, B, T, dtype):
    lib = _lib.load()
    _run("l2s_stem_pool_fused", lambda: lib.l2s_stem_pool_fused(
        _ptr(x), int(x.dtype == torch.float32), _ptr(w), _ptr(bias), _ptr(slope), _ptr(y), B, T, x.shape[-2], x.shape[-1],
        dtype, _stream()), flops=2.0 * B * T * 44 * 44 * 64 * 245,
        nbytes=B * T * (88 * 88 * (4 if x.dtype == torch.float32 else 2) + 22 * 22 * 64 * 2))


def stem_pool_fused_u8(frames, w, bias, slope, y, B, T, dtype, crop=88, mean=0.421, std=0.165):
    lib = _lib.load()
    if frames.dtype != torch.uint8 or frames.dim() != 4:
        raise ValueError("frames: uint8 [B,T,Hin,Win]")
    Hin, Win = frames.shape[-2], frames.shape[-1]
    _run("l2s_stem_pool_fused", lambda: lib.l2s_stem_pool_fused_u8(
        _ptr(frames), Hin, Win, crop, mean, std, _ptr(w), _ptr(bias), _ptr(slope), _ptr(y), B, T, dtype, _stream()),
        flops=2.0 * B * T * 44 * 44 * 64 * 245, nbytes=B * T * (crop * crop + 22 * 22 * 64 * 2))


def maxpool2d_3x3s2(x, y, N, H, W, C, dtype):
    _run("l2s_maxpool2d_3x3s2", lambda: _lib.load().l2s_maxpool2d_3x3s2(_ptr(x), _ptr(y), N, H, W, C, dtype, _stream()))


def avgpool_hw(x, y, N, HW, C, dtype):
    _run("l2s_avgpool_hw", lambda: _lib.load().l2s_avgpool_hw(_ptr(x), _ptr(y), N, HW, C, dtype, _stream()))


def layernorm(x, gamma, beta, eps, y, *, M, C, ldx=None, ldy=None, y2=None, ldy2=0, zero_prefix=0, lens=None,
              len_mul=1, mask_T=0, dtype=F16):
    ldx = ldx if ldx is not None else C
    ldy = ldy if ldy is not None else C + zero_prefix
    _run("l2s_layernorm", lambda: _lib.load().l2s_layernorm(_ptr(x), int(x.dtype == torch.float32), ldx, _ptr(gamma), _ptr(beta), eps, _ptr(y),
                                    int(y.dtype == torch.float32), ldy, _ptr(y2), ldy2, M, C, zero_prefix,
                                    _ptr(lens), len_mul, mask_T, dtype, _stream()))


def attention(qkv, out, *, B, T, H, ldq=None, ldo=None, pos=None, ldp=0, bias_u=None, bias_v=None, lens=None,
              len_mul=1, dtype=F16):
    ldq = ldq if ldq is not None else 3 * H * 64
    ldo = ldo if ldo is not None else H * 64
    _run("l2s_attention", lambda: _lib.load().l2s_attention(_ptr(qkv), ldq, _ptr(out), ldo, _ptr(pos), ldp, _ptr(bias_u), _ptr(bias_v),
                                    _ptr(lens), len_mul, B, T, H, dtype, _stream()))


def glu_dwconv_swish(x, w, bias, y, *, B, T, C, k, lens=None, len_mul=1, dtype=F16):
    _run("l2s_glu_dwconv_swish", lambda: _lib.load().l2s_glu_dwconv_swish(_ptr(x), _ptr(w), _ptr(bias), _ptr(y), _ptr(lens), len_mul, B, T, C, k,
                                           dtype, _stream()))


def greedy_decode(logits, tokens, lprobs, score, *, B, T2, V, ldl=None, lens=None, len_mul=1, temperature=1.0,
                  lenpen=1.0):
    ldl = ldl if ldl is not None else V
    _run("l2s_greedy_decode", lambda: _lib.load().l2s_greedy_decode(_ptr(logits), ldl, _ptr(lens), len_mul, B, T2, V, temperature, lenpen,
                                        _ptr(tokens), _ptr(lprobs), _ptr(score), _stream()))


def beam_decode(logits, *, B, T2, V, beam, ldl=None, lens=None, len_mul=1, temperature=1.0, lenpen=1.0):
    lib = _lib.load()
    dev = logits.device
    ldl = ldl if ldl is not None else V
    nbytes = lib.l2s_beam_decode_workspace(B, T2, beam)
    if nbytes == 0:
        raise L2SError("l2s_beam_decode_workspace: bad shape")
    work = torch.empty(nbytes, device=dev, dtype=torch.uint8)
    tokens = torch.empty(B, beam, T2 + 1, device=dev, dtype=torch.int32)
    pos = torch.empty(B, beam, T2 + 1, device=dev, dtype=torch.float32)
    score = torch.empty(B, beam, device=dev, dtype=torch.float32)
    nhyp = torch.empty(B, device=dev, dtype=torch.int32)
    _run("l2s_beam_decode", lambda: lib.l2s_beam_decode(_ptr(_req(logits, torch.float32, "logits")), ldl, _ptr(lens), len_mul, B, T2, V,
                                                          temperature, lenpen, beam, _ptr(work), nbytes, _ptr(tokens), _ptr(pos),
                                                          _ptr(score), _ptr(nhyp), _stream()))
    return tokens, pos, score, nhyp


def ctc_frames(logits, labels, topk_cls, topk_lp, *, B, L, V, K, ldl=None, lens=None, len_mul=1):
    ldl = ldl if ldl is not None else V
    _run("l2s_ctc_frames", lambda: _lib.load().l2s_ctc_frames(
        _ptr(_req(logits, torch.float32, "logits")), ldl, _ptr(lens), len_mul, B, L, V, K, _ptr(_req(labels, torch.int32, "labels")),
        _ptr(topk_cls), _ptr(topk_lp), _stream()))


def ctc_beam_search(topk_cls, topk_lp, workspace, labels, lengths, scores, *, B, L, K, beam, nbest, lens=None, len_mul=1):
    _run("l2s_ctc_beam_search", lambda: _lib.load().l2s_ctc_beam_search(
        _ptr(_req(topk_cls, torch.int32, "topk_cls")), _ptr(_req(topk_lp, torch.float32, "topk_lp")), _ptr(lens), len_mul, B, L, K,
        beam, nbest, _ptr(workspace), workspace.numel() * workspace.element_size(), _ptr(_req(labels, torch.int32, "labels")),
        _ptr(_req(lengths, torch.int32, "lengths")), _ptr(_req(scores, torch.float32, "scores")), _stream()))


def ctc_repeat_labels(x, y, *, B, L, ldx=None, ldy=None, lens=None, len_mul=1):
    _run("l2s_ctc_repeat_labels", lambda: _lib.load().l2s_ctc_repeat_labels(
        _ptr(_req(x, torch.int32, "x")), ldx or x.stride(0), _ptr(lens), len_mul, B, L, _ptr(_req(y, torch.int32, "y")),
        ldy or y.stride(0), _stream()))


def ctc_beam_workspace_bytes(B, L, beam):
    n = _lib.load().l2s_ctc_beam_workspace(B, L, beam)
    if n == 0:
        raise L2SError(f"l2s_ctc_beam_workspace: unsupported size (B={B}, L={L}, beam={beam})")
    return n


def ctc_decode(logits, *, B, L, V, ldl=None, lens=None, len_mul=1, beam=0, K=40, nbest=3):
    dev = logits.device
    labels = torch.empty(B, L, device=dev, dtype=torch.int32)
    if beam <= 0:
        ctc_frames(logits, labels, None, None, B=B, L=L, V=V, K=0, ldl=ldl, lens=lens, len_mul=len_mul)
        return {"text": labels}
    K = min(K, V)
    nbest = min(nbest, beam)
    tc = torch.empty(B, L, K, device=dev, dtype=torch.int32)
    tl = torch.empty(B, L, K, device=dev, dtype=torch.float32)
    ctc_frames(logits, labels, tc, tl, B=B, L=L, V=V, K=K, ldl=ldl, lens=lens, len_mul=len_mul)
    work = torch.empty(ctc_beam_workspace_bytes(B, L, beam) // 8, device=dev, dtype=torch.int64)
    beams = torch.empty(B, nbest, L, device=dev, dtype=torch.int32)
    blen = torch.empty(B, nbest, device=dev, dtype=torch.int32)
    bsc = torch.empty(B, nbest, device=dev, dtype=torch.float32)
    ctc_beam_search(tc, tl, work, beams, blen, bsc, B=B, L=L, K=K, beam=beam, nbest=nbest, lens=lens, len_mul=len_mul)
    return {"text": labels, "text_beams": beams, "text_lens": blen, "text_scores": bsc}


def repeat2_cast(x, y, B, T, C, dtype):
    _run("l2s_repeat2_cast", lambda: _lib.load().l2s_repeat2_cast(_ptr(x), _ptr(y), B, T, C, dtype, _stream()))


def splitk_reduce(P, x, *, M, N, S, ldp=None, ldx=None):
    _run("l2s_splitk_reduce", lambda: _lib.load().l2s_splitk_reduce(_ptr(P), ldp or S * N, S, _ptr(x), ldx or N, M, N, _stream()))


SPLITK_MAX_M = 512
_SPLITK_ON = os.environ.get("L2S_SPLITK", "1") != "0"


def splitk_slices(M, N, K):
    if not _SPLITK_ON or M > SPLITK_MAX_M or K < 1024 or (N & 63):
        return 0
    S = 8
    while S > 1 and (K % (S * 64) or K // S < 256):
        S //= 2
    return S if S > 1 else 0


def splitk_reduce_layernorm(P, x, gamma, beta, eps, y, *, M, C, S, ldp=None, ldx=None, ldy=None, lens=None, len_mul=1, mask_T=0,
                            dtype=F16):
    _run("l2s_splitk_reduce_layernorm", lambda: _lib.load().l2s_splitk_reduce_layernorm(
        _ptr(P), ldp or S * C, S, _ptr(x), ldx or C, _ptr(gamma), _ptr(beta), eps, _ptr(y), int(y.dtype == torch.float32), ldy or C,
        M, C, _ptr(lens), len_mul, mask_T, dtype, _stream()))


def residual_linear(A, W, bias, x, *, M, N, K, dtype, alpha=1.0, cache=None, key=None, ln=None):
    S = 0 if dtype == F32 else splitk_slices(M, N, K)
    if not S:
        tapgemm(A, W, x, M=M, N=N, Cin=K, bias=bias, alpha=alpha, R=x, ldr=N, flags=F_RES_POST, dtype=dtype)
        if ln is not None:
            layernorm(x, ln[0], ln[1], ln[2], ln[3], M=M, C=N, dtype=dtype)
        return
    ck = (key, S)
    if cache is None or ck not in cache:
        ws = W.view(N, S, K // S).permute(1, 0, 2).contiguous()
        bs = torch.zeros(S * N, device=W.device, dtype=torch.float32)
        if bias is not None:
            bs[:N] = bias
        if cache is not None:
            cache[ck] = (ws, bs)
    else:
        ws, bs = cache[ck]
    P = torch.empty(M, S * N, device=x.device, dtype=torch.float32)
    tapgemm(A, ws, P, M=M, N=N, Cin=K // S, lda=K, ldc=S * N, bias=bs, alpha=alpha, groups=S, a_gstride=K // S, c_gstride=N,
            w_gstride=N * (K // S), dtype=dtype)
    if ln is not None and N in (512, 1024):
        splitk_reduce_layernorm(P, x, ln[0], ln[1], ln[2], ln[3], M=M, C=N, S=S, dtype=dtype)
        return
    splitk_reduce(P, x, M=M, N=N, S=S)
    if ln is not None:
        layernorm(x, ln[0], ln[1], ln[2], ln[3], M=M, C=N, dtype=dtype)


def cast_f32_to_16(x, y, M, C, dtype, ldx=None, ldy=None):
    _run("l2s_cast_f32_to_16", lambda: _lib.load().l2s_cast_f32_to_16(_ptr(x), ldx or C, _ptr(y), ldy or C, M, C, dtype, _stream()))


def cast_16_to_f32(x, y, M, C, dtype, ldx=None, ldy=None):
    _run("l2s_cast_16_to_f32", lambda: _lib.load().l2s_cast_16_to_f32(_ptr(x), ldx or C, _ptr(y), ldy or C, M, C, dtype, _stream()))


def broadcast_rows(v, y, *, B, T, C, ldy, col0=0, ldv=None, lens=None, len_mul=1, dtype=F16):
    _run("l2s_broadcast_rows", lambda: _lib.load().l2s_broadcast_rows(_ptr(v), ldv or C, _ptr(y), ldy, col0, _ptr(lens), len_mul, B, T, C,
                                         int(v.dtype == torch.float32), dtype, _stream()))


def transpose_ct_to_tc(x, y, *, B, C, T, ldy, col0=0, lens=None, len_mul=1, dtype=F16):
    _run("l2s_transpose_ct_to_tc", lambda: _lib.load().l2s_transpose_ct_to_tc(_ptr(x), _ptr(y), ldy, col0, _ptr(lens), len_mul, B, C, T, dtype,
                                             _stream()))


def embedding(code, table, y, *, B, L, C, ldy=None, lens=None, dtype=F16):
    _run("l2s_embedding", lambda: _lib.load().l2s_embedding(_ptr(code), _ptr(table), _ptr(y), ldy or C, _ptr(lens), B, L, C, dtype, _stream()))


def embedding_tokens(tok, table, y, *, B, L, C, token_offset=4, ldt=None, ldy=None, lens=None, len_mul=1, dtype=F16):
    _run("l2s_embedding_tokens", lambda: _lib.load().l2s_embedding_tokens(
        _ptr(tok), ldt or tok.shape[-1], token_offset, _ptr(table), table.shape[0], _ptr(y), ldy or C, _ptr(lens), len_mul, B, L, C,
        dtype, _stream()))


def rows_f32_to_16_masked(x, y, *, B, T, C, ldx=None, ldy=None, col0=0, lens=None, len_mul=1, dtype=F16):
    _run("l2s_rows_f32_to_16_masked", lambda: _lib.load().l2s_rows_f32_to_16_masked(
        _ptr(x), ldx or C, _ptr(y), ldy or C, col0, _ptr(lens), len_mul, B, T, C, dtype, _stream()))


def lens_from_mask(padding_mask, B, T, device):
    import torch
    lens = torch.empty(B, device=device, dtype=torch.int32)
    if padding_mask is not None:
        assert padding_mask.dtype == torch.bool and padding_mask.shape == (B, T) and padding_mask.is_contiguous()
    _run("l2s_lens_from_mask", lambda: _lib.load().l2s_lens_from_mask(_ptr(padding_mask), _ptr(lens), B, T, _stream()))
    return lens


def basicblock_fused(x, w1, b1, s1, w2, b2, s2, y, *, n_images, H, W, C=64, dtype=F16):
    M = float(n_images) * H * W
    _run("l2s_basicblock_fused", lambda: _lib.load().l2s_basicblock_fused(
        _ptr(x), _ptr(w1), _ptr(b1), _ptr(s1), _ptr(w2), _ptr(b2), _ptr(s2), _ptr(y), n_images, H, W, C, dtype, _stream()),
        flops=2.0 * 2 * M * C * C * 9, nbytes=2 * 2 * M * C)


def basicstage128_tail_fused(x0, t0, wa, ba, sa, w1, b1, s1, w2, b2, s2, y, *, n_images, H, W, dtype=F16):
    M = float(n_images) * H * W
    _run("l2s_basicstage128_tail_fused", lambda: _lib.load().l2s_basicstage128_tail_fused(
        _ptr(x0), _ptr(t0), _ptr(wa), _ptr(ba), _ptr(sa), _ptr(w1), _ptr(b1), _ptr(s1), _ptr(w2), _ptr(b2), _ptr(s2), _ptr(y),
        n_images, H, W, dtype, _stream()),
        flops=2.0 * M * 128 * (3 * 9 * 128 + 64), nbytes=2 * M * (128 + 64 + 128))


def basiclayer_fused(x, ws, biases, slopes, y, *, n_images, H, W, C=64, dtype=F16):
    n = len(ws)
    if n % 2 or len(biases) != n or len(slopes) != n:
        raise L2SError("basiclayer_fused: 2 * n_blocks weights, biases and slopes")
    wp = (ctypes.c_void_p * n)(*[_ptr(_req(w, _TORCH16[dtype], "w")) for w in ws])
    bp = (ctypes.c_void_p * n)(*[_ptr(_req(b_, torch.float32, "bias")) for b_ in biases])
    sp = (ctypes.c_void_p * n)(*[_ptr(_req(s_, torch.float32, "slope")) for s_ in slopes])
    M = float(n_images) * H * W
    _run("l2s_basiclayer_fused", lambda: _lib.load().l2s_basiclayer_fused(
        _ptr(x), wp, bp, sp, n // 2, _ptr(y), n_images, H, W, C, dtype, _stream()),
        flops=2.0 * n * M * C * C * 9, nbytes=2 * 2 * M * C)


def split_hi_lo(x, hi, lo, *, B, T, C, act=0, slope=0.0, ldx=None, ld16=None, lens=None, len_mul=1, dtype=F16):
    _run("l2s_split_hi_lo", lambda: _lib.load().l2s_split_hi_lo(_ptr(x), ldx or C, _ptr(hi), _ptr(lo), ld16 or C, act, float(slope),
                                                                _ptr(lens), len_mul, B, T, C, dtype, _stream()))


def conv_post_tanh(x, w, bias, wav, pcm, *, B, T, C, k, lens=None, len_mul=1):
    _run("l2s_conv_post_tanh", lambda: _lib.load().l2s_conv_post_tanh(_ptr(x), _ptr(w), float(bias), _ptr(wav), _ptr(pcm), _ptr(lens), len_mul, B,
                                         T, C, k, _stream()))


def resblock_fused(xl, w, bias, xs, xl_out, *, B, T, C, k, dil, accumulate, slope, lens=None, len_mul=1, dtype=F16):
    _run(f"l2s_resblock_fused<C{C},k{k}>", lambda: _lib.load().l2s_resblock_fused(
        _ptr(xl), _ptr(w), _ptr(bias), _ptr(xs), _ptr(xl_out), _ptr(lens), len_mul, B, T, C, k, dil[0], dil[1], dil[2],
        int(bool(accumulate)), float(slope), dtype, _stream()),
        flops=2.0 * B * T * C * C * k * 6, nbytes=B * T * C * (2 + 4 + (4 if accumulate else 0) + (2 if xl_out is not None else 0)))


def resstage_fused(xl, ws, biases, xs, xl_out, *, B, T, C, ks, dils, slope, lens=None, len_mul=1, dtype=F16, xs_final=True):
    n = len(ws)
    wp = (ctypes.c_void_p * n)(*[_ptr(_req(w, _TORCH16[dtype], "w")) for w in ws])
    bp = (ctypes.c_void_p * n)(*[_ptr(_req(b_, torch.float32, "bias")) for b_ in biases])
    kk = (ctypes.c_int * n)(*[int(k) for k in ks])
    dd = (ctypes.c_int * (3 * n))(*[int(d) for dl in dils for d in dl])
    if xs.dtype != torch.float32:
        raise L2SError("xs must be fp32")
    _run(f"l2s_resstage_fused<C{C}>", lambda: _lib.load().l2s_resstage_fused(
        _ptr(_req(xl, _TORCH16[dtype], "xl")), wp, bp, kk, dd, n, _ptr(xs), _ptr(xl_out), _ptr(lens), len_mul, B, T, C,
        float(slope), int(bool(xs_final)), dtype, _stream()),
        flops=sum(2.0 * B * T * C * C * k * 6 for k in ks),
        nbytes=B * T * C * (2 + (4 if xs_final else 0) + (2 if xl_out is not None else 0)))


def respair(x_l, w1, b1, w2, b2, *, B, T, C, k, dil, slope, y=None, xs=None, accumulate=False, lens=None, len_mul=1, dtype=F16,
            xs_final=True):
    lib = _lib.load()
    d = _lib.RespairDesc()
    d.X, d.W1, d.W2, d.b1, d.b2 = _ptr(_req(x_l, _TORCH16[dtype], "x_l")), _ptr(w1), _ptr(w2), _ptr(_req(b1, torch.float32, "b1")), _ptr(_req(b2, torch.float32, "b2"))
    d.Y, d.XS, d.lens = _ptr(y), _ptr(xs), _ptr(lens)
    if xs is not None and xs.dtype != torch.float32:
        raise L2SError("xs must be fp32")
    if lens is not None and lens.dtype != torch.int32:
        raise L2SError("lens must be int32")
    d.len_mul, d.B, d.T, d.C, d.k, d.dil = len_mul, B, T, C, k, dil
    d.last = 0 if xs is None else (1 if xs_final else 2)
    d.accumulate, d.dtype, d.slope = int(bool(accumulate)), dtype, float(slope)
    kind = "last" if xs is not None else "mid"
    arrays = 2 * 2 + (0 if xs is None else (4 if accumulate else 0) + (4 if xs_final else 0) - (0 if y is not None else 2))
    key = f"l2s_respair<C{C},{kind}>"
    if _profiler is not None and _profiler.detail:
        key += f" k{k} dil{dil}"
    _run(key, lambda: lib.l2s_respair(ctypes.byref(d), _stream()),
         flops=2.0 * B * T * C * C * k * 2, nbytes=float(B) * T * C * arrays + 2.0 * 2 * C * C * k, shape=f"M{B * T} k{k}")


def respair_final(xs_l, w1s, b1s, w2s, b2s, y, *, B, T, C, ks, dils, slope, lens=None, len_mul=1, dtype=F16):
    lib = _lib.load()
    n = len(xs_l)
    if not (1 <= n <= 3 and len(w1s) == len(w2s) == len(b1s) == len(b2s) == len(ks) == len(dils) == n):
        raise L2SError("respair_final: 1..3 ResBlocks, one entry per list each")
    d = _lib.RespairFinalDesc()
    for j in range(n):
        d.X[j], d.W1[j], d.W2[j] = _ptr(_req(xs_l[j], _TORCH16[dtype], "x_l")), _ptr(w1s[j]), _ptr(w2s[j])
        d.b1[j], d.b2[j] = _ptr(_req(b1s[j], torch.float32, "b1")), _ptr(_req(b2s[j], torch.float32, "b2"))
        d.k[j], d.dil[j] = int(ks[j]), int(dils[j])
    if lens is not None and lens.dtype != torch.int32:
        raise L2SError("lens must be int32")
    d.Y, d.lens = _ptr(_req(y, _TORCH16[dtype], "y")), _ptr(lens)
    d.n, d.len_mul, d.B, d.T, d.C, d.dtype, d.slope = n, len_mul, B, T, C, dtype, float(slope)
    _run(f"l2s_respair_final<C{C}>", lambda: lib.l2s_respair_final(ctypes.byref(d), _stream()),
         flops=sum(2.0 * B * T * C * C * k * 2 for k in ks), nbytes=float(B) * T * C * 2 * (n + 1) + sum(2.0 * 2 * C * C * k for k in ks),
         shape=f"M{B * T} n{n}")


def preprocess_frames(frames, y, *, B, T, Hin, Win, crop=88, mean=0.421, std=0.165, dtype=F16):
    _run("l2s_preprocess_frames", lambda: _lib.load().l2s_preprocess_frames(_ptr(frames), _ptr(y), B, T, Hin, Win, crop, mean, std, dtype, _stream()))


def mel_spectrogram(wav, mel, basis, fb, fb_range, *, B, S, T_rows, n_samples=None, ldw=None, ldm=None, n_fft=640, hop=160, n_mels=80,
                    floor=1e-5):
    if wav.dtype not in (torch.float32, torch.int16):
        raise L2SError(f"wav: expected float32 or int16, got {wav.dtype}")
    if n_samples is not None and n_samples.dtype != torch.int32:
        raise L2SError("n_samples must be int32")
    _req(wav, None, "wav"), _req(mel, torch.float32, "mel"), _req(basis, torch.float32, "basis"), _req(fb, torch.float32, "fb")
    _req(fb_range, torch.int32, "fb_range")
    frames = float(B) * T_rows
    _run("l2s_mel_spectrogram", lambda: _lib.load().l2s_mel_spectrogram(
        _ptr(wav), int(wav.dtype == torch.int16), ldw if ldw is not None else S, _ptr(n_samples), B, S, _ptr(basis), _ptr(fb),
        _ptr(fb_range), _ptr(mel), ldm if ldm is not None else n_mels, T_rows, n_fft, hop, n_mels, float(floor), _stream()),
        flops=2.0 * frames * n_fft * n_fft, nbytes=float(B) * S * wav.element_size() + 4.0 * frames * n_mels + 4.0 * n_fft * n_fft)


def unit_ce(logits, target, nll, smooth, n_correct, n_tok, *, B, T2, V, ldl=None, ldt=None, lens=None, len_mul=2, pad_idx=1,
            ignore_prefix=0):
    _req(logits, torch.float32, "logits"), _req(target, torch.int32, "target"), _req(nll, torch.float32, "nll")
    _req(smooth, torch.float32, "smooth"), _req(n_correct, torch.int32, "n_correct"), _req(n_tok, torch.int32, "n_tok")
    if lens is not None:
        _req(lens, torch.int32, "lens")
    ldl = ldl if ldl is not None else V
    ldt = ldt if ldt is not None else target.stride(0)
    if min(nll.numel(), smooth.numel(), n_correct.numel(), n_tok.numel()) < B or (lens is not None and lens.numel() < B):
        raise L2SError("unit_ce: per-clip tensors shorter than B")
    if (B * T2 - 1) * ldl + V > _extent(logits):
        raise L2SError("unit_ce: logits smaller than B*T2 rows of ldl")
    if (B - 1) * ldt + min(T2, ldt) > _extent(target):
        raise L2SError("unit_ce: target smaller than [B, ldt]")
    _run("l2s_unit_ce", lambda: _lib.load().l2s_unit_ce(
        _ptr(logits), ldl, _ptr(target), ldt, _ptr(lens), len_mul, B, T2, V, pad_idx, ignore_prefix, _ptr(nll), _ptr(smooth),
        _ptr(n_correct), _ptr(n_tok), _stream()), nbytes=4.0 * B * T2 * V)


def mel_l1_sc(pred, targ, l1, sq, tsq, n_rows, *, B, Tm_pred, Tm_targ, crop_len, lens=None, len_mul=4, n_mels=80):
    _req(pred, torch.float32, "pred"), _req(targ, torch.float32, "targ")
    for t, n in ((l1, "l1"), (sq, "sq"), (tsq, "tsq")):
        _req(t, torch.float32, n)
    _req(n_rows, torch.int32, "n_rows")
    if lens is not None:
        _req(lens, torch.int32, "lens")
    if not pred.is_contiguous() or not targ.is_contiguous():
        raise L2SError("mel_l1_sc: pred and targ must be dense")
    if pred.numel() < B * Tm_pred * n_mels or targ.numel() < B * Tm_targ * n_mels:
        raise L2SError("mel_l1_sc: pred / targ smaller than [B, Tm, n_mels]")
    if min(l1.numel(), sq.numel(), tsq.numel(), n_rows.numel()) < B or (lens is not None and lens.numel() < B):
        raise L2SError("mel_l1_sc: per-clip tensors shorter than B")
    _run("l2s_mel_l1_sc", lambda: _lib.load().l2s_mel_l1_sc(
        _ptr(pred), Tm_pred, _ptr(targ), Tm_targ, _ptr(lens), len_mul, B, n_mels, crop_len, _ptr(l1), _ptr(sq), _ptr(tsq),
        _ptr(n_rows), _stream()), nbytes=8.0 * B * min(Tm_pred, Tm_targ) * n_mels)


def ctc_loss_workspace_bytes(B, L, S_max):
    n = _lib.load().l2s_ctc_loss_workspace(B, L, S_max)
    if n == 0:
        raise L2SError(f"l2s_ctc_loss_workspace: unsupported size (B={B}, L={L}, S_max={S_max}; at most 511 labels per clip)")
    return n


def ctc_loss(logits, targets, tgt_lens, tgt_offs, workspace, nll, *, B, L, V, S_max, blank=0, ldl=None, lens=None, len_mul=2):
    _req(logits, torch.float32, "logits"), _req(targets, torch.int32, "targets"), _req(tgt_lens, torch.int32, "tgt_lens")
    _req(tgt_offs, torch.int32, "tgt_offs"), _req(nll, torch.float32, "nll")
    if lens is not None:
        _req(lens, torch.int32, "lens")
    ldl = ldl if ldl is not None else V
    if (B * L - 1) * ldl + V > _extent(logits):
        raise L2SError("ctc_loss: logits smaller than B*L rows of ldl")
    if min(tgt_lens.numel(), tgt_offs.numel(), nll.numel()) < B or (lens is not None and lens.numel() < B):
        raise L2SError("ctc_loss: per-clip tensors shorter than B")
    _run("l2s_ctc_loss", lambda: _lib.load().l2s_ctc_loss(
        _ptr(logits), ldl, _ptr(lens), len_mul, B, L, V, blank, _ptr(targets) if targets.numel() else None, _ptr(tgt_lens),
        _ptr(tgt_offs), S_max, _ptr(workspace), workspace.numel() * workspace.element_size(), _ptr(nll), _stream()),
        nbytes=4.0 * B * L * V)


_TG = ("(Tensor A, Tensor W, Tensor(a!) C, *, int M, int N, int Cin, int ntaps=1, int? lda=None, int? ldc=None, Tensor? bias=None, "
       "Tensor? slope=None, Tensor? R=None, int? ldr=None, Tensor(b!)? C2=None, int? ldc2=None, Tensor? lens=None, int mode=0, "
       "int T_out=0, int T_in=0, int stride=1, int dil=1, int off=0, int Ho=0, int Wo=0, int Hi=0, int Wi=0, int KW=1, int pad=0, "
       "int out_row_mul=1, int out_row_add=0, int mask_T=0, int mask_mul=1, int act=0, int flags=0, int dtype=0, float alpha=1.0, "
       "float act_slope=0.0, float slope2=0.0, int groups=1, int a_gstride=0, int c_gstride=0, int w_gstride=0, Tensor? ktab=None, "
       "float? kflops=None) -> ()")
_ATT = ("(Tensor qkv, Tensor(a!) out, *, int B, int T, int H, int? ldq=None, int? ldo=None, Tensor? pos=None, int ldp=0, "
        "Tensor? bias_u=None, Tensor? bias_v=None, Tensor? lens=None, int len_mul=1, int dtype=0) -> ()")
_STEM = "(Tensor x, Tensor w, Tensor bias, Tensor? slope, Tensor(a!) y, int B, int T, int dtype) -> ()"
_RP = ("(Tensor x_l, Tensor w1, Tensor b1, Tensor w2, Tensor b2, *, int B, int T, int C, int k, int dil, float slope, "
       "Tensor(a!)? y=None, Tensor(b!)? xs=None, bool accumulate=False, Tensor? lens=None, int len_mul=1, int dtype=0, "
       "bool xs_final=True) -> ()")
_CPT = ("(Tensor x, Tensor w, float bias, Tensor(a!) wav, Tensor(b!)? pcm, *, int B, int T, int C, int k, Tensor? lens=None, "
        "int len_mul=1) -> ()")
_GLU = ("(Tensor x, Tensor w, Tensor bias, Tensor(a!) y, *, int B, int T, int C, int k, Tensor? lens=None, int len_mul=1, "
        "int dtype=0) -> ()")
_LN = ("(Tensor x, Tensor gamma, Tensor beta, float eps, Tensor(a!) y, *, int M, int C, int? ldx=None, int? ldy=None, "
       "Tensor(b!)? y2=None, int ldy2=0, int zero_prefix=0, Tensor? lens=None, int len_mul=1, int mask_T=0, int dtype=0) -> ()")
_GD = ("(Tensor logits, Tensor(a!) tokens, Tensor(b!) lprobs, Tensor(c!) score, *, int B, int T2, int V, int? ldl=None, "
       "Tensor? lens=None, int len_mul=1, float temperature=1.0, float lenpen=1.0) -> ()")
_BL = "(Tensor x, Tensor[] ws, Tensor[] biases, Tensor[] slopes, Tensor(a!) y, *, int n_images, int H, int W, int C=64, int dtype=0) -> ()"
_SCHEMAS = {
    "tapgemm": _TG,
    "stem_conv3d": _STEM,
    "stem_pool_fused": _STEM,
    "stem_pool_fused_u8": "(Tensor frames, Tensor w, Tensor bias, Tensor? slope, Tensor(a!) y, int B, int T, int dtype, int crop=88, "
                          "float mean=0.421, float std=0.165) -> ()",
    "maxpool2d_3x3s2": "(Tensor x, Tensor(a!) y, int N, int H, int W, int C, int dtype) -> ()",
    "avgpool_hw": "(Tensor x, Tensor(a!) y, int N, int HW, int C, int dtype) -> ()",
    "layernorm": _LN,
    "attention": _ATT,
    "glu_dwconv_swish": _GLU,
    "greedy_decode": _GD,
    "beam_decode": "(Tensor logits, *, int B, int T2, int V, int beam, int? ldl=None, Tensor? lens=None, int len_mul=1, "
                   "float temperature=1.0, float lenpen=1.0) -> (Tensor, Tensor, Tensor, Tensor)",
    "repeat2_cast": "(Tensor x, Tensor(a!) y, int B, int T, int C, int dtype) -> ()",
    "ctc_frames": "(Tensor logits, Tensor(a!) labels, Tensor(b!)? topk_cls, Tensor(c!)? topk_lp, *, int B, int L, int V, int K, "
                  "int? ldl=None, Tensor? lens=None, int len_mul=1) -> ()",
    "ctc_repeat_labels": "(Tensor x, Tensor(a!) y, *, int B, int L, int? ldx=None, int? ldy=None, Tensor? lens=None, "
                         "int len_mul=1) -> ()",
    "ctc_beam_search": "(Tensor topk_cls, Tensor topk_lp, Tensor(a!) workspace, Tensor(b!) labels, Tensor(c!) lengths, "
                       "Tensor(d!) scores, *, int B, int L, int K, int beam, int nbest, Tensor? lens=None, int len_mul=1) -> ()",
    "splitk_reduce": "(Tensor P, Tensor(a!) x, *, int M, int N, int S, int? ldp=None, int? ldx=None) -> ()",
    "splitk_reduce_layernorm": "(Tensor P, Tensor(a!) x, Tensor gamma, Tensor beta, float eps, Tensor(b!) y, *, int M, int C, int S, "
                               "int? ldp=None, int? ldx=None, int? ldy=None, Tensor? lens=None, int len_mul=1, int mask_T=0, int dtype=0) -> ()",
    "cast_f32_to_16": "(Tensor x, Tensor(a!) y, int M, int C, int dtype, int? ldx=None, int? ldy=None) -> ()",
    "cast_16_to_f32": "(Tensor x, Tensor(a!) y, int M, int C, int dtype, int? ldx=None, int? ldy=None) -> ()",
    "broadcast_rows": "(Tensor v, Tensor(a!) y, *, int B, int T, int C, int ldy, int col0=0, int? ldv=None, Tensor? lens=None, "
                      "int len_mul=1, int dtype=0) -> ()",
    "transpose_ct_to_tc": "(Tensor x, Tensor(a!) y, *, int B, int C, int T, int ldy, int col0=0, Tensor? lens=None, int len_mul=1, "
                          "int dtype=0) -> ()",
    "embedding": "(Tensor code, Tensor table, Tensor(a!) y, *, int B, int L, int C, int? ldy=None, Tensor? lens=None, int dtype=0) -> ()",
    "embedding_tokens": "(Tensor tok, Tensor table, Tensor(a!) y, *, int B, int L, int C, int token_offset=4, int? ldt=None, "
                        "int? ldy=None, Tensor? lens=None, int len_mul=1, int dtype=0) -> ()",
    "rows_f32_to_16_masked": "(Tensor x, Tensor(a!) y, *, int B, int T, int C, int? ldx=None, int? ldy=None, int col0=0, "
                             "Tensor? lens=None, int len_mul=1, int dtype=0) -> ()",
    "lens_from_mask": "(Tensor? padding_mask, int B, int T, Device device) -> Tensor",
    "basicblock_fused": "(Tensor x, Tensor w1, Tensor b1, Tensor s1, Tensor w2, Tensor b2, Tensor s2, Tensor(a!) y, *, int n_images, "
                        "int H, int W, int C=64, int dtype=0) -> ()",
    "basiclayer_fused": _BL,
    "basicstage128_tail_fused": "(Tensor x0, Tensor t0, Tensor wa, Tensor ba, Tensor sa, Tensor w1, Tensor b1, Tensor s1, Tensor w2, "
                                "Tensor b2, Tensor s2, Tensor(a!) y, *, int n_images, int H, int W, int dtype=0) -> ()",
    "split_hi_lo": "(Tensor x, Tensor(a!) hi, Tensor(b!) lo, *, int B, int T, int C, int act=0, float slope=0.0, int? ldx=None, "
                   "int? ld16=None, Tensor? lens=None, int len_mul=1, int dtype=0) -> ()",
    "conv_post_tanh": _CPT,
    "resblock_fused": "(Tensor xl, Tensor w, Tensor bias, Tensor(a!) xs, Tensor(b!)? xl_out, *, int B, int T, int C, int k, int[] dil, "
                      "bool accumulate, float slope, Tensor? lens=None, int len_mul=1, int dtype=0) -> ()",
    "resstage_fused": "(Tensor xl, Tensor[] ws, Tensor[] biases, Tensor(a!) xs, Tensor(b!)? xl_out, *, int B, int T, int C, int[] ks, "
                      "int[] dils, float slope, Tensor? lens=None, int len_mul=1, int dtype=0, bool xs_final=True) -> ()",
    "respair": _RP,
    "respair_final": "(Tensor[] xs_l, Tensor[] w1s, Tensor[] b1s, Tensor[] w2s, Tensor[] b2s, Tensor(a!) y, *, int B, int T, int C, int[] ks, "
                     "int[] dils, float slope, Tensor? lens=None, int len_mul=1, int dtype=0) -> ()",
    "preprocess_frames": "(Tensor frames, Tensor(a!) y, *, int B, int T, int Hin, int Win, int crop=88, float mean=0.421, "
                         "float std=0.165, int dtype=0) -> ()",
    "mel_spectrogram": "(Tensor wav, Tensor(a!) mel, Tensor basis, Tensor fb, Tensor fb_range, *, int B, int S, int T_rows, "
                       "Tensor? n_samples=None, int? ldw=None, int? ldm=None, int n_fft=640, int hop=160, int n_mels=80, "
                       "float floor=1e-05) -> ()",
    "unit_ce": "(Tensor logits, Tensor target, Tensor(a!) nll, Tensor(b!) smooth, Tensor(c!) n_correct, Tensor(d!) n_tok, *, int B, "
               "int T2, int V, int? ldl=None, int? ldt=None, Tensor? lens=None, int len_mul=2, int pad_idx=1, "
               "int ignore_prefix=0) -> ()",
    "mel_l1_sc": "(Tensor pred, Tensor targ, Tensor(a!) l1, Tensor(b!) sq, Tensor(c!) tsq, Tensor(d!) n_rows, *, int B, int Tm_pred, "
                 "int Tm_targ, int crop_len, Tensor? lens=None, int len_mul=4, int n_mels=80) -> ()",
    "ctc_loss": "(Tensor logits, Tensor targets, Tensor tgt_lens, Tensor tgt_offs, Tensor(a!) workspace, Tensor(b!) nll, *, int B, "
                "int L, int V, int S_max, int blank=0, int? ldl=None, Tensor? lens=None, int len_mul=2) -> ()",
}
ENTRY_OF = {n: "l2s_" + n for n in _SCHEMAS}
ENTRY_OF.update({"maxpool2d_3x3s2": "l2s_maxpool2d_3x3s2", "avgpool_hw": "l2s_avgpool_hw"})
HOST_QUERIES = ("l2s_abi_version", "l2s_build_info", "l2s_tapgemm_variant", "l2s_tapgemm_epilogue_family", "l2s_beam_decode_workspace",
                "l2s_ctc_beam_workspace", "l2s_ctc_loss_workspace")
ALIASES = {"frontend3d_stem": "stem_pool_fused", "resnet_trunk": "basiclayer_fused", "linear_epilogue": "tapgemm",
           "posconv_gelu": "tapgemm", "convtranspose1d": "tapgemm", "mel_head": "tapgemm", "mhsa_padmask": "attention",
           "relpos_mhsa": "attention", "conformer_conv_module": "glu_dwconv_swish", "greedy_unit_decode": "greedy_decode",
           "resblock1": "respair", "tanh_to_int16": "conv_post_tanh"}

_TORCH_LIB = torch.library.Library("lip2speech", "DEF")


def _fake_none(*a, **k):
    return None


def _fake_beam_decode(logits, *, B, T2, V, beam, ldl=None, lens=None, len_mul=1, temperature=1.0, lenpen=1.0):
    return (logits.new_empty((B, beam, T2 + 1), dtype=torch.int32), logits.new_empty((B, beam, T2 + 1), dtype=torch.float32),
            logits.new_empty((B, beam), dtype=torch.float32), logits.new_empty((B,), dtype=torch.int32))


def _fake_lens_from_mask(padding_mask, B, T, device):
    return torch.empty(B, device=device, dtype=torch.int32)


def _resstage_fused_flat(xl, ws, biases, xs, xl_out, *, B, T, C, ks, dils, slope, lens=None, len_mul=1, dtype=F16, xs_final=True):
    return _IMPL["resstage_fused"](xl, ws, biases, xs, xl_out, B=B, T=T, C=C, ks=ks, dils=[dils[i:i + 3] for i in range(0, len(dils), 3)],
                                   slope=slope, lens=lens, len_mul=len_mul, dtype=dtype, xs_final=xs_final)


_IMPL = {}


def _register_torch_ops():
    g = globals()
    for name, schema in _SCHEMAS.items():
        _IMPL[name] = g[name]
    for name, schema in _SCHEMAS.items():
        impl = _resstage_fused_flat if name == "resstage_fused" else _IMPL[name]
        fake = {"beam_decode": _fake_beam_decode, "lens_from_mask": _fake_lens_from_mask}.get(name, _fake_none)
        for op in [name] + [a for a, base in ALIASES.items() if base == name]:
            _TORCH_LIB.define(op + schema)
            _TORCH_LIB.impl(op, impl, "CompositeExplicitAutograd" if name == "lens_from_mask" else "CUDA")
            torch.library.register_fake("lip2speech::" + op)(fake)

    def router(name):
        op = getattr(torch.ops.lip2speech, name)

        def call(*a, **k):
            try:
                return op(*a, **k)
            except NotImplementedError as e:
                raise L2SError(f"lip2speech::{name}: HIP ops need device tensors (there is no CPU path)") from e
        call.__name__ = name
        call.__doc__ = _IMPL[name].__doc__
        return call
    for name in _SCHEMAS:
        if name == "resstage_fused":
            op = torch.ops.lip2speech.resstage_fused

            def resstage_fused(xl, ws, biases, xs, xl_out, *, B, T, C, ks, dils, slope, lens=None, len_mul=1, dtype=F16, xs_final=True):
                try:
                    return op(xl, list(ws), list(biases), xs, xl_out, B=B, T=T, C=C, ks=[int(k) for k in ks],
                              dils=[int(d) for dl in dils for d in dl], slope=slope, lens=lens, len_mul=len_mul, dtype=dtype,
                              xs_final=xs_final)
                except NotImplementedError as e:
                    raise L2SError("lip2speech::resstage_fused: HIP ops need device tensors (there is no CPU path)") from e
            resstage_fused.__doc__ = _IMPL[name].__doc__
            g[name] = resstage_fused
        else:
            g[name] = router(name)


_register_torch_ops()
```

Measured before the change: 13580 audio-sec/wall-sec.

## Fuse residual LayerNorm into the phase GEMM tail using per-band completion counters

```diff
diff --git a/include/lip2speech_hip.h b/include/lip2speech_hip.h
--- a/include/lip2speech_hip.h
+++ b/include/lip2speech_hip.h
@@ -125,6 +125,11 @@
                                 void* y, int y_is_f32, int ldy, int M, int C, const int32_t* lens, int len_mul, int mask_T,
                                 int dtype, void* stream);
 
+int l2s_residual_linear_ln(const l2s_gemm_desc* host_desc, const float* gamma, const float* beta, float eps, void* y, int y_is_f32,
+                           int ldy, const float* gamma2, const float* beta2, float eps2, void* y2, int ldy2, const int32_t* lens,
+                           int len_mul, int mask_T, int32_t* counters, void* stream);
+int l2s_residual_linear_ln_supported(int M, int N, int K, int dtype);
+
 int l2s_cast_f32_to_16(const float* x, int ldx, void* y, int ldy, int M, int C, int dtype, void* stream);
 int l2s_cast_16_to_f32(const void* x, int ldx, float* y, int ldy, int M, int C, int dtype, void* stream);
 int l2s_broadcast_rows(const void* v, int ldv, void* y, int ldy, int col0, const int32_t* lens, int len_mul,
diff --git a/lip2speech_unit_amd/_lib.py b/lip2speech_unit_amd/_lib.py
--- a/lip2speech_unit_amd/_lib.py
+++ b/lip2speech_unit_amd/_lib.py
@@ -81,6 +81,8 @@
     "l2s_repeat2_cast": ([_vp, _vp, _i, _i, _i, _i, _vp], _i),
     "l2s_splitk_reduce": ([_vp, _i, _i, _vp, _i, _i, _i, _vp], _i),
     "l2s_splitk_reduce_layernorm": ([_vp, _i, _i, _vp, _i, _vp, _vp, _f, _vp, _i, _i, _i, _i, _vp, _i, _i, _i, _vp], _i),
+    "l2s_residual_linear_ln": ([ctypes.POINTER(GemmDesc), _vp, _vp, _f, _vp, _i, _i, _vp, _vp, _f, _vp, _i, _vp, _i, _i, _vp, _vp], _i),
+    "l2s_residual_linear_ln_supported": ([_i, _i, _i, _i], _i),
     "l2s_cast_f32_to_16": ([_vp, _i, _vp, _i, _i, _i, _i, _vp], _i),
     "l2s_cast_16_to_f32": ([_vp, _i, _vp, _i, _i, _i, _i, _vp], _i),
     "l2s_broadcast_rows": ([_vp, _i, _vp, _i, _i, _vp, _i, _i, _i, _i, _i, _i, _vp], _i),
diff --git a/lip2speech_unit_amd/conformer.py b/lip2speech_unit_amd/conformer.py
--- a/lip2speech_unit_amd/conformer.py
+++ b/lip2speech_unit_amd/conformer.py
@@ -215,12 +215,16 @@
         glu_in = torch.empty(M, 2 * d, device=dev, dtype=t16)
         cv = torch.empty(M, d, device=dev, dtype=t16)
 
-        def half_ffn(e, name, norm, after, y):
+        cnt = ops.ln_counters(M, dev) if (ops.ln_inlaunch(M, d, d, dt) or ops.ln_inlaunch(M, d, F, dt)) else None
+
+        def half_ffn(e, name, norm, after, y, after2=None):
             w = e[name]
-            ops.layernorm(x, norm[0], norm[1], 1e-12, h, M=M, C=d, dtype=dt)
+            if norm is not None:
+                ops.layernorm(x, norm[0], norm[1], 1e-12, h, M=M, C=d, dtype=dt)
             ops.tapgemm(h, w[0], f, M=M, N=F, Cin=d, bias=w[1], act=ACT_RELU, dtype=dt)
             ops.residual_linear(f, w[2], w[3], x, M=M, N=d, K=F, alpha=0.5, dtype=dt, cache=e, key=name,
-                                ln=(after[0], after[1], 1e-12, y))
+                                ln=(after[0], after[1], 1e-12, y),
+                                ln2=None if after2 is None else (after2[0], after2[1], 1e-12, h), counters=cnt)
 
         for li, e in enumerate(P["layers"] if self.raven else ()):
             ops.layernorm(x, e["n_mha"][0], e["n_mha"][1], 1e-12, h, M=M, C=d, dtype=dt)
@@ -232,17 +236,20 @@
             w = e["ff"]
             ops.tapgemm(h, w[0], f, M=M, N=F, Cin=d, bias=w[1], act=ACT_RELU, dtype=dt)
             ops.tapgemm(f, w[2], x, M=M, N=d, Cin=F, bias=w[3], R=x, ldr=d, flags=F_RES_POST, dtype=dt)
-        for li, e in enumerate(() if self.raven else P["layers"]):
-            half_ffn(e, "ffm", e["n_ffm"], e["n_mha"], h)
+        layers = () if self.raven else P["layers"]
+        for li, e in enumerate(layers):
+            half_ffn(e, "ffm", e["n_ffm"] if li == 0 else None, e["n_mha"], h)
             ops.tapgemm(h, e["wqkv"], qkv, M=M, N=3 * d, Cin=d, bias=e["bqkv"], dtype=dt)
             ops.attention(qkv, att, B=B, T=T, H=H, pos=pos[:, li * d:], ldp=nl * d, bias_u=e["u"], bias_v=e["v"],
                           lens=lens, len_mul=len_mul, dtype=dt)
-            ops.tapgemm(att, e["wo"], x, M=M, N=d, Cin=d, bias=e["bo"], R=x, ldr=d, flags=F_RES_POST, dtype=dt)
-            ops.layernorm(x, e["n_conv"][0], e["n_conv"][1], 1e-12, h, M=M, C=d, dtype=dt)
+            ops.residual_linear(att, e["wo"], e["bo"], x, M=M, N=d, K=d, dtype=dt, cache=e, key="wo",
+                                ln=(e["n_conv"][0], e["n_conv"][1], 1e-12, h), counters=cnt)
             ops.tapgemm(h, e["pw1"], glu_in, M=M, N=2 * d, Cin=d, bias=e["pb1"], dtype=dt)
             ops.glu_dwconv_swish(glu_in, e["dw"], e["db"], cv, B=B, T=T, C=d, k=k, lens=lens, len_mul=len_mul, dtype=dt)
-            ops.tapgemm(cv, e["pw2"], x, M=M, N=d, Cin=d, bias=e["pb2"], R=x, ldr=d, flags=F_RES_POST, dtype=dt)
-            half_ffn(e, "ff", e["n_ff"], e["n_fin"], x)
+            ops.residual_linear(cv, e["pw2"], e["pb2"], x, M=M, N=d, K=d, dtype=dt, cache=e, key="pw2",
+                                ln=(e["n_ff"][0], e["n_ff"][1], 1e-12, h), counters=cnt)
+            nxt = layers[li + 1]["n_ffm"] if li + 1 < len(layers) else None
+            half_ffn(e, "ff", None, e["n_fin"], x, after2=nxt)
         return x
 
 
diff --git a/lip2speech_unit_amd/csrc/layernorm_rows.h b/lip2speech_unit_amd/csrc/layernorm_rows.h
--- /dev/null
+++ b/lip2speech_unit_amd/csrc/layernorm_rows.h
@@ -0,0 +1,134 @@
+#pragma once
+#include "l2s_common.h"
+
+namespace l2s {
+
+template <int VPL, int ROWS, bool GUARD = true>
+__device__ __forceinline__ void ln_rows_load(float4 (&v)[ROWS][VPL], const float* x, const int ldx, const int row0, const int M,
+                                             const int lane) {
+#pragma unroll
+  for (int r = 0; r < ROWS; ++r)
+#pragma unroll
+    for (int i = 0; i < VPL; ++i) {
+      v[r][i] = make_float4(0.f, 0.f, 0.f, 0.f);
+      if (!GUARD || row0 + r < M) v[r][i] = *reinterpret_cast<const float4*>(x + (int64_t)(row0 + r) * ldx + (i * 64 + lane) * 4);
+    }
+}
+
+template <int VPL>
+__device__ __forceinline__ void ln_params_load(float4 (&g)[VPL], float4 (&bt)[VPL], const float* gamma, const float* beta,
+                                               const int lane) {
+#pragma unroll
+  for (int i = 0; i < VPL; ++i) {
+    g[i] = *reinterpret_cast<const float4*>(gamma + (i * 64 + lane) * 4);
+    bt[i] = *reinterpret_cast<const float4*>(beta + (i * 64 + lane) * 4);
+  }
+}
+
+template <typename ET, int VPL, int ROWS, bool YF32, bool KEEP, bool GUARD = true>
+__device__ __forceinline__ void ln_rows_finish(float4 (&v)[ROWS][VPL], const float4 (&g)[VPL], const float4 (&bt)[VPL],
+                                               const float eps, void* y, const int ldy, const int row0, const int M,
+                                               const int32_t* lens, const int len_mul, const int mask_T, const int lane) {
+  static_assert(!KEEP || YF32, "a second LayerNorm reads the fp32 result of the first");
+  constexpr int C = VPL * 256;
+  float mean[ROWS], rstd[ROWS];
+#pragma unroll
+  for (int r = 0; r < ROWS; ++r) {
+    float s = 0.f;
+#pragma unroll
+    for (int i = 0; i < VPL; ++i) s += (v[r][i].x + v[r][i].y) + (v[r][i].z + v[r][i].w);
+    mean[r] = s;
+  }
+#pragma unroll
+  for (int o = 32; o > 0; o >>= 1)
+#pragma unroll
+    for (int r = 0; r < ROWS; ++r) mean[r] += __shfl_xor(mean[r], o, 64);
+#pragma unroll
+  for (int r = 0; r < ROWS; ++r) {
+    mean[r] *= (1.0f / (float)C);
+    float q = 0.f;
+#pragma unroll
+    for (int i = 0; i < VPL; ++i) {
+      const float a = v[r][i].x - mean[r], b = v[r][i].y - mean[r], c = v[r][i].z - mean[r], d = v[r][i].w - mean[r];
+      q += (a * a + b * b) + (c * c + d * d);
+    }
+    rstd[r] = q;
+  }
+#pragma unroll
+  for (int o = 32; o > 0; o >>= 1)
+#pragma unroll
+    for (int r = 0; r < ROWS; ++r) rstd[r] += __shfl_xor(rstd[r], o, 64);
+#pragma unroll
+  for (int r = 0; r < ROWS; ++r) {
+    const int row = row0 + r;
+    if (GUARD && row >= M) break;
+    const float rs = rsqrtf(rstd[r] * (1.0f / (float)C) + eps);
+    bool keep = true;
+    if (lens) {
+      const int clip = row / mask_T;
+      keep = (row - clip * mask_T) < lens[clip] * len_mul;
+    }
+#pragma unroll
+    for (int i = 0; i < VPL; ++i) {
+      float4 o = make_float4((v[r][i].x - mean[r]) * rs * g[i].x + bt[i].x, (v[r][i].y - mean[r]) * rs * g[i].y + bt[i].y,
+                             (v[r][i].z - mean[r]) * rs * g[i].z + bt[i].z, (v[r][i].w - mean[r]) * rs * g[i].w + bt[i].w);
+      if (!keep) o = make_float4(0.f, 0.f, 0.f, 0.f);
+      if (YF32) {
+        *reinterpret_cast<float4*>((float*)y + (int64_t)row * ldy + (i * 64 + lane) * 4) = o;
+        if (KEEP) v[r][i] = o;
+      } else {
+        const uint32_t lo = ET::pack2(o.x, o.y), hi = ET::pack2(o.z, o.w);
+        const uint32_t nlo = __shfl_xor(lo, 1, 64), nhi = __shfl_xor(hi, 1, 64);
+        if (!(lane & 1))
+          *reinterpret_cast<uint4*>((uint16_t*)y + (int64_t)row * ldy + (i * 64 + lane) * 4) = make_uint4(lo, hi, nlo, nhi);
+      }
+    }
+  }
+}
+
+struct LnTail {
+  const float* gamma;
+  const float* beta;
+  void* y;
+  const float* gamma2;
+  const float* beta2;
+  void* y2;
+  const int32_t* lens;
+  int32_t* counters;
+  float eps, eps2;
+  int ldy, ldy2, y_f32, len_mul, mask_T;
+};
+struct NoLnTail {};
+
+template <typename ET, int VPL, bool YF32, bool LN2>
+__device__ __forceinline__ void ln_band_pass(const LnTail& t, const float* x, const int ldx, const int r_lo, const int M,
+                                             const int lane) {
+  constexpr int ROWS = VPL == 4 ? 2 : 4;
+  constexpr int NB = 8 / ROWS;
+  const int r_hi = r_lo + 32 < M ? r_lo + 32 : M;
+  if (r_lo >= r_hi) return;
+  float4 g[VPL], bt[VPL], g2[LN2 ? VPL : 1], bt2[LN2 ? VPL : 1];
+  ln_params_load<VPL>(g, bt, t.gamma, t.beta, lane);
+  if constexpr (LN2) ln_params_load<VPL>(g2, bt2, t.gamma2, t.beta2, lane);
+  for (int row0 = r_lo; row0 < r_hi; row0 += 8) {
+    float4 v[NB][ROWS][VPL];
+#pragma unroll
+    for (int k = 0; k < NB; ++k) ln_rows_load<VPL, ROWS, false>(v[k], x, ldx, row0 + k * ROWS, M, lane);
+#pragma unroll
+    for (int k = 0; k < NB; ++k) {
+      ln_rows_finish<ET, VPL, ROWS, YF32, LN2, false>(v[k], g, bt, t.eps, t.y, t.ldy, row0 + k * ROWS, M, t.lens, t.len_mul,
+                                                      t.mask_T, lane);
+      if constexpr (LN2) {
+#pragma unroll
+        for (int r = 0; r < ROWS; ++r)
+#pragma unroll
+          for (int i = 0; i < VPL; ++i)
+            asm volatile("" : "+v"(v[k][r][i].x), "+v"(v[k][r][i].y), "+v"(v[k][r][i].z), "+v"(v[k][r][i].w));
+        ln_rows_finish<ET, VPL, ROWS, false, false, false>(v[k], g2, bt2, t.eps2, t.y2, t.ldy2, row0 + k * ROWS, M, nullptr, 1, 1,
+                                                           lane);
+      }
+    }
+  }
+}
+
+}
diff --git a/lip2speech_unit_amd/csrc/phasegemm.hip b/lip2speech_unit_amd/csrc/phasegemm.hip
--- a/lip2speech_unit_amd/csrc/phasegemm.hip
+++ b/lip2speech_unit_amd/csrc/phasegemm.hip
@@ -1,5 +1,6 @@
 #include "l2s_common.h"
 #include "tapgemm_tiles.h"
+#include "layernorm_rows.h"
 #include <cstdlib>
 
 int l2s_phasegemm_f16_m0(const l2s_gemm_desc& d, hipStream_t st);
@@ -10,6 +11,8 @@
 int l2s_phasegemm_bf16_m2(const l2s_gemm_desc& d, hipStream_t st);
 int l2s_phasegemm_f16_m3(const l2s_gemm_desc& d, hipStream_t st);
 int l2s_phasegemm_bf16_m3(const l2s_gemm_desc& d, hipStream_t st);
+int l2s_phasegemm_f16_ln(const l2s_gemm_desc& d, const l2s::LnTail& ln, hipStream_t st);
+int l2s_phasegemm_bf16_ln(const l2s_gemm_desc& d, const l2s::LnTail& ln, hipStream_t st);
 
 int l2s_phasegemm_ktab_launch(const l2s_gemm_desc& d, hipStream_t st) {
   if (d.mode != L2S_MODE_LINEAR || d.groups < 1) return L2S_EINVAL;
@@ -69,3 +72,58 @@
     default: return L2S_EINVAL;
   }
 }
+
+static l2s_gemm_desc residual_desc(int M, int N, int K, int dtype) {
+  l2s_gemm_desc d = {};
+  d.M = M; d.N = N; d.Cin = K; d.ntaps = 1;
+  d.lda = K; d.ldc = d.ldr = d.ldc2 = N;
+  d.mode = L2S_MODE_LINEAR;
+  d.out_row_mul = 1; d.mask_mul = 1;
+  d.flags = L2S_F_RES_POST | L2S_F_RES_F32 | L2S_F_OUT_F32;
+  d.dtype = dtype; d.alpha = 1.f; d.groups = 1;
+  return d;
+}
+
+extern "C" int l2s_residual_linear_ln_supported(int M, int N, int K, int dtype) {
+  if (dtype != L2S_F16 && dtype != L2S_BF16) return 0;
+  if (N != 512 && N != 1024) return 0;
+  if (M <= 0 || K <= 0) return 0;
+  return l2s_phasegemm_eligible(residual_desc(M, N, K, dtype)) ? 1 : 0;
+}
+
+extern "C" int l2s_residual_linear_ln(const l2s_gemm_desc* hd, const float* gamma, const float* beta, float eps, void* y,
+                                      int y_is_f32, int ldy, const float* gamma2, const float* beta2, float eps2, void* y2,
+                                      int ldy2, const int32_t* lens, int len_mul, int mask_T, int32_t* counters, void* stream) {
+  if (!hd || !hd->A || !hd->W || !hd->C || !hd->R || !gamma || !beta || !y || !counters) return L2S_EINVAL;
+  l2s_gemm_desc d = *hd;
+  if (d.M <= 0 || d.N <= 0 || d.Cin <= 0) return L2S_ESHAPE;
+  if (d.groups <= 0) d.groups = 1;
+  if (d.out_row_mul <= 0) d.out_row_mul = 1;
+  if (lens && (len_mul <= 0 || mask_T <= 0)) return L2S_EINVAL;
+  const bool two = gamma2 || beta2 || y2;
+  if (two && (!gamma2 || !beta2 || !y2)) return L2S_EINVAL;
+  if (d.dtype == L2S_F32) return L2S_EUNSUPPORTED;
+  if (d.dtype != L2S_F16 && d.dtype != L2S_BF16) return L2S_EINVAL;
+  if (d.N != 512 && d.N != 1024) return L2S_EUNSUPPORTED;
+  if (d.mode != L2S_MODE_LINEAR || d.ntaps != 1 || d.groups != 1 || d.ktab || d.act != L2S_ACT_NONE ||
+      d.flags != (L2S_F_RES_POST | L2S_F_RES_F32 | L2S_F_OUT_F32) || d.R != d.C || d.ldr != d.ldc || d.out_row_mul != 1 ||
+      d.out_row_add != 0)
+    return L2S_EUNSUPPORTED;
+  if (two && !y_is_f32) return L2S_EUNSUPPORTED;
+  if (d.ldc < d.N || ldy < d.N || (two && ldy2 < d.N)) return L2S_ESHAPE;
+  if ((d.Cin & 7) || (d.lda & 7) || (d.ldc & 3) || ((uintptr_t)d.A & 15) || ((uintptr_t)d.W & 15) || ((uintptr_t)d.C & 15))
+    return L2S_EALIGN;
+  if ((ldy & (y_is_f32 ? 3 : 7)) || ((uintptr_t)y & 15) || (two && ((ldy2 & 7) || ((uintptr_t)y2 & 15))) || ((uintptr_t)counters & 3))
+    return L2S_EALIGN;
+  if (y == d.A || (two && (y2 == d.A || y2 == y))) return L2S_EINVAL;
+  if (!y_is_f32 && y == d.C) return L2S_EINVAL;
+  if (!l2s_phasegemm_eligible(d)) return L2S_EUNSUPPORTED;
+  l2s::LnTail t = {};
+  t.gamma = gamma; t.beta = beta; t.y = y;
+  t.gamma2 = two ? gamma2 : nullptr; t.beta2 = two ? beta2 : nullptr; t.y2 = two ? y2 : nullptr;
+  t.lens = lens; t.counters = counters;
+  t.eps = eps; t.eps2 = eps2;
+  t.ldy = ldy; t.ldy2 = ldy2; t.y_f32 = y_is_f32 ? 1 : 0; t.len_mul = len_mul; t.mask_T = mask_T;
+  hipStream_t st = (hipStream_t)stream;
+  return d.dtype == L2S_F16 ? l2s_phasegemm_f16_ln(d, t, st) : l2s_phasegemm_bf16_ln(d, t, st);
+}
diff --git a/lip2speech_unit_amd/csrc/phasegemm_inst.hip b/lip2speech_unit_amd/csrc/phasegemm_inst.hip
--- a/lip2speech_unit_amd/csrc/phasegemm_inst.hip
+++ b/lip2speech_unit_amd/csrc/phasegemm_inst.hip
@@ -12,6 +12,14 @@
 
 int L2S_INST_NAME(const l2s_gemm_desc& d, hipStream_t st) { return launch_phase_mode<InstET, L2S_INST_MODE>(d, st); }
 
+#if L2S_INST_MODE == 0
+#if L2S_INST_ET == 0
+int l2s_phasegemm_f16_ln(const l2s_gemm_desc& d, const l2s::LnTail& ln, hipStream_t st) { return launch_phase_ln<InstET>(d, ln, st); }
+#else
+int l2s_phasegemm_bf16_ln(const l2s_gemm_desc& d, const l2s::LnTail& ln, hipStream_t st) { return launch_phase_ln<InstET>(d, ln, st); }
+#endif
+#endif
+
 #if defined(L2S_PHASE_STAMPS) && L2S_INST_ET == 0 && L2S_INST_MODE == 0
 extern "C" int l2s_debug_phase_stamps(void* buf) { return phase_set_stamps(buf); }
 #endif
diff --git a/lip2speech_unit_amd/csrc/phasegemm_kernel.h b/lip2speech_unit_amd/csrc/phasegemm_kernel.h
--- a/lip2speech_unit_amd/csrc/phasegemm_kernel.h
+++ b/lip2speech_unit_amd/csrc/phasegemm_kernel.h
@@ -1,5 +1,6 @@
 #pragma once
 #include "tapgemm_common.h"
+#include "layernorm_rows.h"
 #include <cstdlib>
 
 using namespace l2s;
@@ -20,9 +21,11 @@
 #endif
 
 constexpr int PG_KTAB = 3;
-template <typename ET, int MODE_T, int EPI>
+template <typename ET, int MODE_T, int EPI, int LNV = 0>
 __global__ __launch_bounds__(512) void phasegemm_kernel(const l2s_gemm_desc p, const int tilesM, const int tilesN,
-                                                        const int chunk, const int band) {
+                                                        const int chunk, const int band,
+                                                        const std::conditional_t<(LNV > 0), LnTail, NoLnTail> ln) {
+  static_assert(LNV == 0 || (MODE_T == (int)L2S_MODE_LINEAR && EPI == L2S_EPI_S32), "the LayerNorm tail rides on the S32 family");
   constexpr bool KT = MODE_T == PG_KTAB;
   constexpr int MODE = KT ? (int)L2S_MODE_LINEAR : MODE_T;
   constexpr int MI = 8, NI = 4;
@@ -373,6 +376,38 @@
       epilogue_stream32x<ET, MI, NI>(p, acc, lane, m0 + wr * 128, n0 + wc * 64, rowmap);
     } else if constexpr (EPI == L2S_EPI_S32) {
       epilogue_direct32<ET, MI, NI>(p, acc, lane, m0 + wr * 128, n0 + wc * 64, grp, rowmap);
+      if constexpr (LNV > 0) {
+        const uint32_t last_w = lds_base + 8 * Q_B;
+        wait_vmcnt<0>();
+        __builtin_amdgcn_s_barrier();
+        if (wave == 4) {
+          int old = 0;
+          if (lane == 0) {
+            __builtin_amdgcn_fence(__ATOMIC_RELEASE, "agent");
+            asm volatile("s_waitcnt vmcnt(0)" ::: "memory");
+            old = __hip_atomic_fetch_add(ln.counters + (m0 >> 8), 1, __ATOMIC_RELAXED, __HIP_MEMORY_SCOPE_AGENT);
+          }
+          old = __builtin_amdgcn_readfirstlane(old);
+          const int is_last = ((old + 1) % tilesN) == 0 ? 1 : 0;
+          if (is_last && lane == 0) {
+            __builtin_amdgcn_fence(__ATOMIC_ACQUIRE, "agent");
+            asm volatile("s_waitcnt vmcnt(0)" ::: "memory");
+          }
+          asm volatile("ds_write_b32 %0, %1\n\ts_waitcnt lgkmcnt(0)" ::"v"(last_w), "v"(is_last) : "memory");
+        }
+        __builtin_amdgcn_s_barrier();
+        if (wr == 0) __builtin_amdgcn_s_barrier();
+        int last_v;
+        asm volatile("ds_read_b32 %0, %1\n\ts_waitcnt lgkmcnt(0)" : "=v"(last_v) : "v"(last_w) : "memory");
+        if (__builtin_amdgcn_readfirstlane(last_v)) {
+          const float* xs = (const float*)p.C;
+          const int r_lo = m0 + wave * 32;
+          if (ln.gamma2) ln_band_pass<ET, LNV, true, true>(ln, xs, p.ldc, r_lo, p.M, lane);
+          else if (ln.y_f32) ln_band_pass<ET, LNV, true, false>(ln, xs, p.ldc, r_lo, p.M, lane);
+          else ln_band_pass<ET, LNV, false, false>(ln, xs, p.ldc, r_lo, p.M, lane);
+        }
+        if (wr == 1) __builtin_amdgcn_s_barrier();
+      }
     } else if constexpr (PAIRED) {
       epilogue_direct16<ET, MI, NI, EPI, decltype(rowmap), NoHook, true>(p, acc, lane, m0 + wr * 128, n0 + wc * 64, grp, rowmap);
     } else if constexpr (EPI == L2S_EPI_G16A) {
@@ -401,9 +436,9 @@
 #endif
 }
 
-template <typename ET, int MODE, int EPI>
-int launch_phase(const l2s_gemm_desc& d, hipStream_t st) {
-  auto kern = phasegemm_kernel<ET, MODE, EPI>;
+template <typename ET, int MODE, int EPI, int LNV = 0>
+int launch_phase(const l2s_gemm_desc& d, hipStream_t st, const std::conditional_t<(LNV > 0), LnTail, NoLnTail> ln = {}) {
+  auto kern = phasegemm_kernel<ET, MODE, EPI, LNV>;
   static L2sSmemOptIn opt_in;
   if (int e = l2s_smem_opt_in(kern, p_smem(EPI), opt_in)) return e;
   const int tilesM = (d.M + PBM - 1) / PBM, tilesN = (d.N + PBN - 1) / PBN;
@@ -420,9 +455,18 @@
     const double fp = ap * (an < tilesM ? an : tilesM) + wp * wn;
     if (fp < best) { best = fp; band = b; }
   }
-  hipLaunchKernelGGL(kern, dim3(8 * slots), dim3(512), p_smem(EPI), st, d, tilesM, tilesN, chunk, band);
+  static const int band_env = [] { const char* e = getenv("L2S_BAND"); return e ? atoi(e) : 0; }();
+  if (band_env > 0) band = band_env < tilesM ? band_env : tilesM;
+  hipLaunchKernelGGL(kern, dim3(8 * slots), dim3(512), p_smem(EPI), st, d, tilesM, tilesN, chunk, band, ln);
   L2S_CHECK_LAUNCH();
   return L2S_OK;
+}
+
+template <typename ET>
+int launch_phase_ln(const l2s_gemm_desc& d, const LnTail& ln, hipStream_t st) {
+  if (d.N == 1024) return launch_phase<ET, (int)L2S_MODE_LINEAR, L2S_EPI_S32, 4>(d, st, ln);
+  if (d.N == 512) return launch_phase<ET, (int)L2S_MODE_LINEAR, L2S_EPI_S32, 2>(d, st, ln);
+  return L2S_EUNSUPPORTED;
 }
 
 
diff --git a/lip2speech_unit_amd/hubert.py b/lip2speech_unit_amd/hubert.py
--- a/lip2speech_unit_amd/hubert.py
+++ b/lip2speech_unit_amd/hubert.py
@@ -146,6 +146,7 @@
         att = torch.empty(M, d, device=dev, dtype=t16)
         f = torch.empty(M, F, device=dev, dtype=t16)
         out = torch.empty(M, d, device=dev, dtype=torch.float32)
+        cnt = ops.ln_counters(M, dev) if (ops.ln_inlaunch(M, d, d, dt) or ops.ln_inlaunch(M, d, F, dt)) else None
         layers = P["layers"]
         if not layers:
             ops.layernorm(x, P["lnf"][0], P["lnf"][1], 1e-5, out, M=M, C=d, dtype=dt)
@@ -155,12 +156,12 @@
             ops.tapgemm(h, e["wqkv"], qkv, M=M, N=3 * d, Cin=d, bias=e["bqkv"], dtype=dt)
             ops.attention(qkv, att, B=B, T=T, H=H, lens=lens, len_mul=1, dtype=dt)
             ops.residual_linear(att, e["wo"], e["bo"], x, M=M, N=d, K=d, dtype=dt, cache=e, key="wo",
-                                ln=(e["ln2"][0], e["ln2"][1], 1e-5, h))
+                                ln=(e["ln2"][0], e["ln2"][1], 1e-5, h), counters=cnt)
             ops.tapgemm(h, e["w1"], f, M=M, N=F, Cin=d, bias=e["b1"], act=ACT_GELU, dtype=dt)
             last = li + 1 == len(layers)
             nxt = P["lnf"] if last else layers[li + 1]["ln1"]
             ops.residual_linear(f, e["w2"], e["b2"], x, M=M, N=d, K=F, dtype=dt, cache=e, key="w2",
-                                ln=(nxt[0], nxt[1], 1e-5, out if last else h))
+                                ln=(nxt[0], nxt[1], 1e-5, out if last else h), counters=cnt)
         return out
 
 
diff --git a/lip2speech_unit_amd/ops.py b/lip2speech_unit_amd/ops.py
--- a/lip2speech_unit_amd/ops.py
+++ b/lip2speech_unit_amd/ops.py
@@ -307,12 +307,55 @@
         M, C, _ptr(lens), len_mul, mask_T, dtype, _stream()))
 
 
-def residual_linear(A, W, bias, x, *, M, N, K, dtype, alpha=1.0, cache=None, key=None, ln=None):
+_LN_INLAUNCH = int(os.environ.get("L2S_LN_INLAUNCH", "0"))
+
+
+def ln_inlaunch(M, N, K, dtype) -> bool:
+    if dtype == F32 or not (_LN_INLAUNCH & {512: 1, 1024: 2}.get(N, 0)):
+        return False
+    return bool(_lib.load().l2s_residual_linear_ln_supported(M, N, K, dtype))
+
+
+def ln_counters(M, device):
+    return torch.zeros((M + 255) // 256, device=device, dtype=torch.int32)
+
+
+def residual_linear_ln(A, W, bias, x, gamma, beta, eps, y, counters, *, M, N, K, alpha=1.0, gamma2=None, beta2=None, eps2=0.0,
+                       y2=None, ldy=None, ldy2=None, lens=None, len_mul=1, mask_T=0, dtype=F16):
+    lib = _lib.load()
+    if bias is not None and bias.dtype != torch.float32:
+        raise L2SError("bias must be fp32")
+    if x.dtype != torch.float32 or counters.dtype != torch.int32 or counters.numel() < (M + 255) // 256:
+        raise L2SError("residual_linear_ln: x fp32, counters int32 [(M + 255) // 256]")
+    d = GemmDesc()
+    d.A, d.W, d.C, d.R, d.bias = _ptr(A), _ptr(W), _ptr(x), _ptr(x), _ptr(bias)
+    d.M, d.N, d.Cin, d.ntaps = M, N, K, 1
+    d.lda, d.ldc, d.ldc2, d.ldr = K, N, N, N
+    d.mode, d.out_row_mul, d.mask_mul, d.groups = MODE_LINEAR, 1, 1, 1
+    d.flags, d.act, d.dtype, d.alpha = F_RES_POST | F_RES_F32 | F_OUT_F32, ACT_NONE, dtype, alpha
+    two = y2 is not None
+    nbytes = 2.0 * M * K + 2.0 * N * K + 8.0 * M * N + (4.0 if y.dtype == torch.float32 else 2.0) * M * N + (2.0 * M * N if two else 0.0)
+    _run(f"tapgemm<{_DTYPE_NAME[dtype]},256x256,mode0,e8,ln{N}>", lambda: lib.l2s_residual_linear_ln(
+        ctypes.byref(d), _ptr(gamma), _ptr(beta), eps, _ptr(y), int(y.dtype == torch.float32), ldy or N, _ptr(gamma2), _ptr(beta2),
+        eps2, _ptr(y2), ldy2 or N, _ptr(lens), len_mul, mask_T, _ptr(counters), _stream()),
+        flops=2.0 * M * N * K, nbytes=nbytes, shape=f"M{M} N{N} K{K}")
+
+
+def residual_linear(A, W, bias, x, *, M, N, K, dtype, alpha=1.0, cache=None, key=None, ln=None, ln2=None, counters=None):
+    if ln2 is not None and ln is None:
+        raise L2SError("residual_linear: ln2 is a LayerNorm on the result of ln")
     S = 0 if dtype == F32 else splitk_slices(M, N, K)
     if not S:
+        if ln is not None and counters is not None and ln_inlaunch(M, N, K, dtype):
+            two = ln2 if ln2 is not None else (None, None, 0.0, None)
+            residual_linear_ln(A, W, bias, x, ln[0], ln[1], ln[2], ln[3], counters, M=M, N=N, K=K, alpha=alpha, gamma2=two[0],
+                               beta2=two[1], eps2=two[2], y2=two[3], dtype=dtype)
+            return
         tapgemm(A, W, x, M=M, N=N, Cin=K, bias=bias, alpha=alpha, R=x, ldr=N, flags=F_RES_POST, dtype=dtype)
         if ln is not None:
             layernorm(x, ln[0], ln[1], ln[2], ln[3], M=M, C=N, dtype=dtype)
+        if ln2 is not None:
+            layernorm(ln[3], ln2[0], ln2[1], ln2[2], ln2[3], M=M, C=N, dtype=dtype)
         return
     ck = (key, S)
     if cache is None or ck not in cache:
@@ -329,10 +372,12 @@
             w_gstride=N * (K // S), dtype=dtype)
     if ln is not None and N in (512, 1024):
         splitk_reduce_layernorm(P, x, ln[0], ln[1], ln[2], ln[3], M=M, C=N, S=S, dtype=dtype)
-        return
-    splitk_reduce(P, x, M=M, N=N, S=S)
-    if ln is not None:
-        layernorm(x, ln[0], ln[1], ln[2], ln[3], M=M, C=N, dtype=dtype)
+    else:
+        splitk_reduce(P, x, M=M, N=N, S=S)
+        if ln is not None:
+            layernorm(x, ln[0], ln[1], ln[2], ln[3], M=M, C=N, dtype=dtype)
+    if ln2 is not None:
+        layernorm(ln[3], ln2[0], ln2[1], ln2[2], ln2[3], M=M, C=N, dtype=dtype)
 
 
 def cast_f32_to_16(x, y, M, C, dtype, ldx=None, ldy=None):
@@ -602,6 +647,10 @@
     "splitk_reduce": "(Tensor P, Tensor(a!) x, *, int M, int N, int S, int? ldp=None, int? ldx=None) -> ()",
     "splitk_reduce_layernorm": "(Tensor P, Tensor(a!) x, Tensor gamma, Tensor beta, float eps, Tensor(b!) y, *, int M, int C, int S, "
                                "int? ldp=None, int? ldx=None, int? ldy=None, Tensor? lens=None, int len_mul=1, int mask_T=0, int dtype=0) -> ()",
+    "residual_linear_ln": "(Tensor A, Tensor W, Tensor? bias, Tensor(a!) x, Tensor gamma, Tensor beta, float eps, Tensor(b!) y, "
+                          "Tensor(c!) counters, *, int M, int N, int K, float alpha=1.0, Tensor? gamma2=None, Tensor? beta2=None, "
+                          "float eps2=0.0, Tensor(d!)? y2=None, int? ldy=None, int? ldy2=None, Tensor? lens=None, int len_mul=1, "
+                          "int mask_T=0, int dtype=0) -> ()",
     "cast_f32_to_16": "(Tensor x, Tensor(a!) y, int M, int C, int dtype, int? ldx=None, int? ldy=None) -> ()",
     "cast_16_to_f32": "(Tensor x, Tensor(a!) y, int M, int C, int dtype, int? ldx=None, int? ldy=None) -> ()",
     "broadcast_rows": "(Tensor v, Tensor(a!) y, *, int B, int T, int C, int ldy, int col0=0, int? ldv=None, Tensor? lens=None, "
@@ -645,7 +694,7 @@
 ENTRY_OF = {n: "l2s_" + n for n in _SCHEMAS}
 ENTRY_OF.update({"maxpool2d_3x3s2": "l2s_maxpool2d_3x3s2", "avgpool_hw": "l2s_avgpool_hw"})
 HOST_QUERIES = ("l2s_abi_version", "l2s_build_info", "l2s_tapgemm_variant", "l2s_tapgemm_epilogue_family", "l2s_beam_decode_workspace",
-                "l2s_ctc_beam_workspace", "l2s_ctc_loss_workspace")
+                "l2s_ctc_beam_workspace", "l2s_ctc_loss_workspace", "l2s_residual_linear_ln_supported")
 ALIASES = {"frontend3d_stem": "stem_pool_fused", "resnet_trunk": "basiclayer_fused", "linear_epilogue": "tapgemm",
            "posconv_gelu": "tapgemm", "convtranspose1d": "tapgemm", "mel_head": "tapgemm", "mhsa_padmask": "attention",
            "relpos_mhsa": "attention", "conformer_conv_module": "glu_dwconv_swish", "greedy_unit_decode": "greedy_decode",
```

Measured after the change: 13580 audio-sec/wall-sec, median of 3. About the same (-0.0%).
